# markweberdev/maskbit

Measured on AMD Instinct MI355X. Metric: images/sec (256x256, 64-step MaskBit-12bit, CFG), higher is better.
Workload: dtype f16

## Files before the change

include/maskbit_hip_diag.h:

```cpp
#ifndef MASKBIT_HIP_DIAG_H
#define MASKBIT_HIP_DIAG_H

#include "maskbit_hip.h"

#ifdef __cplusplus
extern "C" {
#endif

int mb_gemm(int epi, const void* A, const void* W, const float* bias, const float* residual, float* out_f32,
            void* out_h16, int M, int N, int K, int period, int variant, mb_stream stream);
int mb_gemm_ex(int epi, const void* A, const void* W, const float* bias, const float* residual, float* out_f32, void* out_h16,
               int M, int N, int K, const float* ln_stats, const float* ln_g, const float* ln_b, int period, int variant, mb_stream stream);
int mb_layernorm(const float* y, const float* gamma, const float* beta, float eps, float* x_f32, void* x_h16, void* x_lo, float* stats,
                 int M, int d, mb_stream stream);
int mb_gemm_act_split(int epi, const void* A_hi, const void* A_lo, const void* W, const float* bias, const float* residual,
                      float* out_f32, void* out_h16, int M, int N, int kw, int variant, mb_stream stream);
int mb_gemm_mini(int epi, const void* A, const void* W, const float* bias, const float* residual, float* out_f32, void* out_h16, void* out4,
                 void* out4_scale, int rows, int pair, int N, int K, int nlo, const void* const* lo, mb_stream stream);
int mb_gemm_mini_seq(int epi, const void* A, const void* W, const float* bias, const float* residual, float* out_f32, void* out_h16, void* out4,
                     void* out4_scale, void* out4l, void* out4l_scale, int rows, int pair, int seq_rows, int N, int K, int nlo, const void* const* lo, mb_stream stream);
int mb_w4_from_f32(const float* W, int N, int K, void* dst4, void* scale_out, mb_stream stream);
int mb_w4lo_from_f32(const float* W, int N, int K, void* dst4, void* scale_out, mb_stream stream);
int mb_gemm_head(int epi, const void* A_hi, const void* A_lo, const void* W_hi, const void* W_lo, const float* scale, const float* bias, int bias_per_pos,
                 float* out_f32, int M, int N, int kw, int period, mb_stream stream);
int mb_cast_f32_to_h16(const float* src, void* dst, int64_t n, mb_stream stream);
int mb_split_f32_planes(const float* src, void* hi, void* lo, int N, int K, float* scale_out, unsigned* tmp, mb_stream stream);
int mb_gemm_mini_split(int epi, const void* A_hi, const void* A_lo, const void* W, const float* bias, void* out_h16, void* out4, void* out4_scale,
                       int rows, int N, int kw, const void* const* lo, mb_stream stream);
int mb_gemm_mini_ln(const void* A, const void* W, const float* bias, float* y, const float* ln_stats, const float* ln_g, const float* ln_b, int rows, int pair,
                    int seq_rows, int N, int K, int nlo, const void* const* lo, mb_stream stream);
int mb_layernorm_f4(const float* y, const float* gamma, const float* beta, float eps, float* x_f32, void* x_h16, void* x4, void* x4_scale, void* xl4,
                    void* xl4_scale, int M, int d, mb_stream stream);
int mb_layernorm_f4_seq(const float* y, const float* gamma, const float* beta, float eps, float* x_f32, void* x_h16, void* x4, void* x4_scale, void* xl4,
                        void* xl4_scale, int M, int d, int seq_rows, mb_stream stream);

int mb_layernorm_pair(const float* y, const float* gamma, const float* beta, float eps, void* x_h16, float* stats, void* x4, void* x4_scale, void* xl4,
                      void* xl4_scale, int P, int d, int seq_rows, mb_stream stream);
int mb_pairify(const float* x_f32, void* x_h16, void* x4, void* x4_scale, void* xl4, void* xl4_scale, int P, int d, int seq_rows, mb_stream stream);
int mb_embed_ln(const int64_t* tokens, const int64_t* labels, const uint8_t* drop, const float* w_in, const float* b_in, const float* class_emb,
                const float* pos, const float* gamma, const float* beta, const float* tables, float* x_f32, void* x_h16, void* x_lo, void* x4,
                void* x4_scale, void* xl4, void* xl4_scale, int nb, int seq, int m, int gbits, int d, int nclass, mb_stream stream);
int mb_embed_pair(const int64_t* tokens, const int64_t* labels, const float* w_in, const float* b_in, const float* class_emb, const float* pos,
                  const float* gamma, const float* beta, const float* tables, float* x_f32, void* x_h16, void* x4, void* x4_scale, void* xl4,
                  void* xl4_scale, int nb, int seq, int m, int gbits, int d, int nclass, mb_stream stream);
int mb_attention_pair(const void* qkv, void* out_h16, int pairs, int N, int d, int heads, mb_stream stream);
int mb_attention_pair_f4(const void* qkv, void* out_h16, void* out4, void* out4_scale, void* out4l, void* out4l_scale, int pairs, int N, int d, int heads, mb_stream stream);
int mb_attention(const void* qkv, void* out_h16, void* out4, void* out4_scale, int nb, int N, int d, int heads, mb_stream stream);
int mb_attention_probs(const void* qkv, float* out_f32, int nb, int N, int d, int heads, mb_stream stream);
int mb_gen_set_alo(mb_gen* g, int gemm_mask);
int mb_set_cu_count(int n);
int mb_gen_set_walk(mb_gen* g, int mode);
int mb_diag_set_walk(int reverse);
int mb_walk_tile(int vb, int ntiles, int reverse);
int mb_walk_seq(int slot, int n, int grp, int reverse);
int mb_walk_row(int slot, int rows, int seq_rows, int pair, int reverse);
int mb_walk_group(int seq_rows, int pair);
int mb_gemm_ht_supported(int epi, int M, int N, int K);

int mb_seeded_noise(const int64_t* seeds, int step, float randomize_temperature, float conf_weight, float* exp_u, float* exp_noise, float* conf_u,
                    float* conf_noise, int B, int P, int C, mb_stream stream);

int mb_vq_argmin(const float* z, const float* codebook, int N, int C, int K, int l2, int splits, int64_t* idx, float* dist, mb_stream stream);

int mb_vq_encode_rows(const void* z_h16, int stride16, const float* z_f32, const float* codebook, int B, int HW, int C, int K, int l2, int splits,
                      int64_t* idx, float* zq_nchw, float* zraw_nchw, float* dist, mb_stream stream);
int mb_vq_gather(const int64_t* codes, const float* codebook, int64_t npix, int C, int K, int l2, int cin_pad, void* out_h16, unsigned* sat,
                 mb_stream stream);
int mb_vq_pack_latent(const float* z_nchw, int B, int K, int HW, int cin_pad, void* out_h16, unsigned* sat, mb_stream stream);
int mb_lfq_pack(const void* z_h16, int B, int HW, int K, int Kp, int64_t* idx, float* zq_nchw, float* zraw_nchw, mb_stream stream);
int mb_lfq_latent(const int64_t* tokens, int64_t npix, int K, void* out_h16, mb_stream stream);
int mb_pack_image(const float* img_nchw, int B, int C, int H, int W, void* out_h16, mb_stream stream);

int mb_conv_layer(const void* in_h16, const float* w_oihw, const float* bias, const float* gn_gamma, const float* gn_beta, const void* residual_h16,
                  void* out_h16, float* img_nchw, uint8_t* img_nhwc_u8, const float* out_gamma, const float* out_beta, float* out_scale_shift,
                  float* out_gn_part, int* part_tiles, unsigned* saturated, int B, int H, int W, int Cin, int Cout, int ks, int up, int final_layer,
                  mb_stream stream);
int mb_groupnorm_stats(const void* x_h16, const float* gamma, const float* beta, float* scale_shift, int B, int HW, int C, mb_stream stream);
int mb_avgpool2(const void* x_h16, void* y_h16, int B, int H, int W, int C, mb_stream stream);
int mb_s2d(const void* x_h16, void* y_h16, int B, int H, int W, int C, mb_stream stream);

int mb_conv_relu_layer(const void* in_h16, const float* w_oihw, const float* bias, void* out_h16, unsigned* saturated, int B, int H, int W, int Cin,
                       int Cout, int ks, mb_stream stream);
int mb_maxpool2(const void* x_h16, void* y_h16, int B, int H, int W, int C, mb_stream stream);
int mb_lpips_input(const float* real, const float* fake, const float* shift_scale, void* out_h16, int B, int H, int W, int clamp01, mb_stream stream);
int mb_lpips_distance(const void* feat_a, const void* feat_b, const float* w, int B, int HW, int C, double* per_image, mb_stream stream);
int mb_lpips_features(mb_lpips* h, const float* real, const float* fake, int B, int H, int W, int clamp01, void* tap0, void* tap1, void* tap2, void* tap3,
                      void* tap4, mb_stream stream);

int mb_convbn_layer(const void* in_h16, const float* w_oihw, const float* scale, const float* shift, void* out_h16, unsigned* saturated, int B, int H,
                    int W, int Cin, int Cout, int kh, int kw, int stride, int ph, int pw, int in_off, int in_cs, int out_off, int out_cs, int variant,
                    mb_stream stream);
int mb_pool3(const void* x_h16, void* y_h16, int B, int H, int W, int C, int mode, int in_off, int in_cs, int out_off, int out_cs, mb_stream stream);
int mb_inception_input(const uint8_t* u8, void* out_h16, int B, int H, int W, mb_stream stream);
int mb_inception_taps(mb_inception* h, const uint8_t* u8, int B, int H, int W, void* map0, void* map1, void* map2, void* map3, float* tap64,
                      float* tap192, float* tap768, float* pool, float* logits_unbiased, float* logits, mb_stream stream);

int mb_spatial_attention(const void* q, const void* k, const void* v, void* out_h16, unsigned* sat, int B, int N, int ld, int ldo, mb_stream stream);
int mb_taming_set_tap(mb_taming* h, int block, void* out_h16);

int mb_gemm_f32(int epi, const float* A, const float* W, const float* bias, const float* residual, float* out, int M, int N, int K, int period,
                int bias_per_pos, mb_stream stream);
int mb_attention_f32(const float* qkv, float* out, int nb, int N, int d, int heads, mb_stream stream);

#ifdef __cplusplus
}
#endif
#endif
```

maskbit_amd/_lib.py:

```python
from __future__ import annotations

import ctypes as C
import os
from typing import Optional

_HERE = os.path.dirname(os.path.abspath(__file__))
LIB_PATH = os.path.join(_HERE, "libmaskbit_hip.so")
ABI_VERSION = 8


class GenCfg(C.Structure):
    _fields_ = [(n, C.c_int) for n in ("bits", "splits", "hidden", "heads", "depth", "mlp", "seq", "nclass", "prenorm", "embed_tables", "precision")]


class DecCfg(C.Structure):
    _fields_ = [("token_size", C.c_int), ("hidden_channels", C.c_int), ("num_resolutions", C.c_int),
                ("num_res_blocks", C.c_int), ("num_channels", C.c_int), ("channel_mult", C.c_int * 8),
                ("latent_size", C.c_int), ("build_encoder", C.c_int), ("sample_with_conv", C.c_int),
                ("enc_res_blocks", C.c_int)]


class SamplePlan(C.Structure):
    _fields_ = [("num_steps", C.c_int), ("use_guidance", C.c_int), ("scale", C.POINTER(C.c_float)),
                ("temperature", C.POINTER(C.c_float)), ("mask_len", C.POINTER(C.c_int)), ("step_begin", C.c_int), ("step_end", C.c_int)]


class EditPlan(C.Structure):
    _fields_ = [("num_steps", C.c_int), ("use_guidance", C.c_int), ("scale", C.POINTER(C.c_float)),
                ("temperature", C.POINTER(C.c_float)), ("mask_ratio", C.POINTER(C.c_float)), ("step_begin", C.c_int), ("step_end", C.c_int)]


class RequestStep(C.Structure):
    _fields_ = [("scale", C.c_float), ("temperature", C.c_float), ("mask_ratio", C.c_float), ("randomize_temperature", C.c_float),
                ("conf_weight", C.c_float), ("step", C.c_int32)]


class RequestPlan(C.Structure):
    _fields_ = [("num_steps", C.c_int), ("use_guidance", C.c_int), ("active", C.POINTER(C.c_int)), ("table", C.c_void_p)]


SIGNATURES = {
    "mb_gen_saturation_count": (C.c_int, [C.c_void_p, C.POINTER(C.c_uint), C.c_int, C.c_void_p]),
    "mb_abi_version": (C.c_int, []),
    "mb_last_error": (C.c_char_p, []),
    "mb_gen_create": (C.c_int, [C.POINTER(GenCfg), C.c_int, C.POINTER(C.c_void_p)]),
    "mb_gen_destroy": (None, [C.c_void_p]),
    "mb_gen_load": (C.c_int, [C.c_void_p, C.c_char_p, C.c_void_p, C.POINTER(C.c_int64), C.c_int, C.c_void_p]),
    "mb_gen_set_alo": (C.c_int, [C.c_void_p, C.c_int]),
    "mb_gen_forward": (C.c_int, [C.c_void_p, C.c_void_p, C.c_void_p, C.c_void_p, C.c_void_p, C.c_int, C.c_void_p]),
    "mb_gen_forward_cfg": (C.c_int, [C.c_void_p, C.c_void_p, C.c_void_p, C.c_void_p, C.c_int, C.c_void_p]),
    "mb_gen_forward_attn": (C.c_int, [C.c_void_p, C.c_void_p, C.c_void_p, C.c_void_p, C.c_void_p, C.c_void_p, C.c_int, C.c_void_p]),
    "mb_sample_step": (C.c_int, [C.c_void_p, C.c_void_p, C.c_float, C.c_float, C.c_void_p, C.c_void_p, C.c_int,
                                 C.c_void_p, C.c_void_p, C.c_void_p, C.c_int, C.c_int, C.c_int, C.c_int, C.c_void_p]),
    "mb_dec_create": (C.c_int, [C.POINTER(DecCfg), C.c_int, C.POINTER(C.c_void_p)]),
    "mb_dec_destroy": (None, [C.c_void_p]),
    "mb_dec_load": (C.c_int, [C.c_void_p, C.c_char_p, C.c_void_p, C.POINTER(C.c_int64), C.c_int, C.c_void_p]),
    "mb_dec_decode": (C.c_int, [C.c_void_p, C.c_void_p, C.c_void_p, C.c_void_p, C.c_int, C.c_void_p]),
    "mb_dec_saturation_count": (C.c_int, [C.c_void_p, C.POINTER(C.c_uint), C.c_int, C.c_void_p]),
    "mb_enc_encode": (C.c_int, [C.c_void_p, C.c_void_p, C.c_void_p, C.c_void_p, C.c_void_p, C.c_int, C.c_void_p]),
    "mb_dec_create_vq": (C.c_int, [C.POINTER(DecCfg), C.c_int, C.c_int, C.c_int, C.POINTER(C.c_void_p)]),
    "mb_dec_decode_latent": (C.c_int, [C.c_void_p, C.c_void_p, C.c_void_p, C.c_void_p, C.c_int, C.c_void_p]),
    "mb_enc_encode_vq": (C.c_int, [C.c_void_p, C.c_void_p, C.c_void_p, C.c_void_p, C.c_void_p, C.c_void_p, C.c_int, C.c_void_p]),
    "mb_vq_argmin": (C.c_int, [C.c_void_p, C.c_void_p, C.c_int, C.c_int, C.c_int, C.c_int, C.c_int, C.c_void_p, C.c_void_p, C.c_void_p]),
    "mb_vq_encode_rows": (C.c_int, [C.c_void_p, C.c_int, C.c_void_p, C.c_void_p] + [C.c_int] * 6 + [C.c_void_p] * 5),
    "mb_vq_gather": (C.c_int, [C.c_void_p, C.c_void_p, C.c_int64, C.c_int, C.c_int, C.c_int, C.c_int, C.c_void_p, C.c_void_p, C.c_void_p]),
    "mb_vq_pack_latent": (C.c_int, [C.c_void_p, C.c_int, C.c_int, C.c_int, C.c_int, C.c_void_p, C.c_void_p, C.c_void_p]),
    "mb_lfq_pack": (C.c_int, [C.c_void_p, C.c_int, C.c_int, C.c_int, C.c_int, C.c_void_p, C.c_void_p, C.c_void_p, C.c_void_p]),
    "mb_lfq_latent": (C.c_int, [C.c_void_p, C.c_int64, C.c_int, C.c_void_p, C.c_void_p]),
    "mb_pack_image": (C.c_int, [C.c_void_p, C.c_int, C.c_int, C.c_int, C.c_int, C.c_void_p, C.c_void_p]),
    "mb_sample": (C.c_int, [C.c_void_p, C.c_void_p, C.POINTER(SamplePlan), C.c_void_p, C.c_int, C.c_void_p, C.c_void_p,
                            C.c_void_p, C.c_void_p, C.c_void_p, C.c_void_p, C.c_void_p]),
    "mb_sample_step_edit": (C.c_int, [C.c_void_p, C.c_void_p, C.c_float, C.c_float, C.c_void_p, C.c_void_p, C.c_float, C.c_void_p,
                                      C.c_void_p, C.c_void_p, C.c_void_p, C.c_int, C.c_int, C.c_int, C.c_int, C.c_void_p]),
    "mb_sample_edit": (C.c_int, [C.c_void_p, C.c_void_p, C.POINTER(EditPlan), C.c_void_p, C.c_int, C.c_void_p, C.c_void_p, C.c_void_p,
                                 C.c_void_p, C.c_void_p, C.c_void_p, C.c_void_p, C.c_void_p]),
    "mb_sample_step_seeded": (C.c_int, [C.c_void_p, C.c_void_p, C.c_float, C.c_float, C.c_void_p, C.c_int, C.c_float, C.c_float, C.c_float, C.c_void_p,
                                        C.c_void_p, C.c_void_p, C.c_void_p, C.c_int, C.c_int, C.c_int, C.c_int, C.c_void_p]),
    "mb_sample_seeded": (C.c_int, [C.c_void_p, C.c_void_p, C.POINTER(EditPlan), C.c_void_p, C.c_int, C.c_void_p, C.c_void_p, C.c_float,
                                   C.POINTER(C.c_float), C.c_void_p, C.c_void_p, C.c_void_p, C.c_void_p, C.c_void_p]),
    "mb_sample_step_requests": (C.c_int, [C.c_void_p, C.c_void_p, C.c_void_p, C.c_void_p, C.c_void_p, C.c_void_p, C.c_void_p, C.c_void_p,
                                          C.c_int, C.c_int, C.c_int, C.c_int, C.c_void_p]),
    "mb_sample_requests": (C.c_int, [C.c_void_p, C.c_void_p, C.POINTER(RequestPlan), C.c_void_p, C.c_int, C.c_void_p, C.c_void_p,
                                     C.c_void_p, C.c_void_p, C.c_void_p, C.c_void_p, C.c_void_p]),
    "mb_seeded_noise": (C.c_int, [C.c_void_p, C.c_int, C.c_float, C.c_float, C.c_void_p, C.c_void_p, C.c_void_p, C.c_void_p, C.c_int, C.c_int, C.c_int,
                                  C.c_void_p]),
    "mb_edit_init": (C.c_int, [C.c_void_p, C.c_void_p, C.c_void_p, C.c_void_p, C.c_int, C.c_int, C.c_int, C.c_int, C.c_void_p]),
    "mb_edit_token_mask": (C.c_int, [C.c_void_p, C.c_void_p, C.c_int, C.c_int, C.c_int, C.c_int, C.c_void_p]),
    "mb_edit_composite": (C.c_int, [C.c_void_p, C.c_void_p, C.c_void_p, C.c_void_p, C.c_void_p, C.c_int, C.c_int, C.c_int, C.c_int, C.c_void_p]),
    "mb_gemm_ex": (C.c_int, [C.c_int, C.c_void_p, C.c_void_p, C.c_void_p, C.c_void_p, C.c_void_p, C.c_void_p, C.c_int, C.c_int, C.c_int,
                             C.c_void_p, C.c_void_p, C.c_void_p, C.c_int, C.c_int, C.c_void_p]),
    "mb_layernorm": (C.c_int, [C.c_void_p, C.c_void_p, C.c_void_p, C.c_float, C.c_void_p, C.c_void_p, C.c_void_p, C.c_void_p, C.c_int, C.c_int, C.c_void_p]),
    "mb_w4_from_f32": (C.c_int, [C.c_void_p, C.c_int, C.c_int, C.c_void_p, C.c_void_p, C.c_void_p]),
    "mb_w4lo_from_f32": (C.c_int, [C.c_void_p, C.c_int, C.c_int, C.c_void_p, C.c_void_p, C.c_void_p]),
    "mb_gemm_head": (C.c_int, [C.c_int, C.c_void_p, C.c_void_p, C.c_void_p, C.c_void_p, C.c_void_p, C.c_void_p, C.c_int, C.c_void_p, C.c_int, C.c_int,
                               C.c_int, C.c_int, C.c_void_p]),
    "mb_cast_f32_to_h16": (C.c_int, [C.c_void_p, C.c_void_p, C.c_int64, C.c_void_p]),
    "mb_split_f32_planes": (C.c_int, [C.c_void_p, C.c_void_p, C.c_void_p, C.c_int, C.c_int, C.c_void_p, C.c_void_p, C.c_void_p]),
    "mb_layernorm_f4": (C.c_int, [C.c_void_p, C.c_void_p, C.c_void_p, C.c_float, C.c_void_p, C.c_void_p, C.c_void_p, C.c_void_p, C.c_void_p, C.c_void_p,
                                  C.c_int, C.c_int, C.c_void_p]),
    "mb_layernorm_f4_seq": (C.c_int, [C.c_void_p, C.c_void_p, C.c_void_p, C.c_float] + [C.c_void_p] * 6 + [C.c_int] * 3 + [C.c_void_p]),
    "mb_layernorm_pair": (C.c_int, [C.c_void_p, C.c_void_p, C.c_void_p, C.c_float] + [C.c_void_p] * 6 + [C.c_int] * 3 + [C.c_void_p]),
    "mb_pairify": (C.c_int, [C.c_void_p] * 6 + [C.c_int] * 3 + [C.c_void_p]),
    "mb_embed_ln": (C.c_int, [C.c_void_p] * 17 + [C.c_int] * 6 + [C.c_void_p]),
    "mb_embed_pair": (C.c_int, [C.c_void_p] * 15 + [C.c_int] * 6 + [C.c_void_p]),
    "mb_attention": (C.c_int, [C.c_void_p, C.c_void_p, C.c_void_p, C.c_void_p, C.c_int, C.c_int, C.c_int, C.c_int, C.c_void_p]),
    "mb_attention_probs": (C.c_int, [C.c_void_p, C.c_void_p, C.c_int, C.c_int, C.c_int, C.c_int, C.c_void_p]),
    "mb_attention_pair": (C.c_int, [C.c_void_p, C.c_void_p, C.c_int, C.c_int, C.c_int, C.c_int, C.c_void_p]),
    "mb_attention_pair_f4": (C.c_int, [C.c_void_p, C.c_void_p, C.c_void_p, C.c_void_p, C.c_void_p, C.c_void_p, C.c_int, C.c_int, C.c_int, C.c_int, C.c_void_p]),
    "mb_gemm_mini": (C.c_int, [C.c_int, C.c_void_p, C.c_void_p, C.c_void_p, C.c_void_p, C.c_void_p, C.c_void_p, C.c_void_p, C.c_void_p, C.c_int, C.c_int,
                               C.c_int, C.c_int, C.c_int, C.POINTER(C.c_void_p), C.c_void_p]),
    "mb_gemm_mini_seq": (C.c_int, [C.c_int, C.c_void_p, C.c_void_p, C.c_void_p, C.c_void_p, C.c_void_p, C.c_void_p, C.c_void_p, C.c_void_p, C.c_void_p, C.c_void_p, C.c_int, C.c_int,
                                   C.c_int, C.c_int, C.c_int, C.c_int, C.POINTER(C.c_void_p), C.c_void_p]),
    "mb_gemm_mini_split": (C.c_int, [C.c_int, C.c_void_p, C.c_void_p, C.c_void_p, C.c_void_p, C.c_void_p, C.c_void_p, C.c_void_p, C.c_int, C.c_int, C.c_int,
                                     C.POINTER(C.c_void_p), C.c_void_p]),
    "mb_gemm_mini_ln": (C.c_int, [C.c_void_p] * 7 + [C.c_int] * 6 + [C.POINTER(C.c_void_p), C.c_void_p]),
    "mb_gemm_act_split": (C.c_int, [C.c_int, C.c_void_p, C.c_void_p, C.c_void_p, C.c_void_p, C.c_void_p, C.c_void_p, C.c_void_p, C.c_int, C.c_int, C.c_int,
                                    C.c_int, C.c_void_p]),
    "mb_gemm": (C.c_int, [C.c_int, C.c_void_p, C.c_void_p, C.c_void_p, C.c_void_p, C.c_void_p, C.c_void_p, C.c_int, C.c_int, C.c_int,
                          C.c_int, C.c_int, C.c_void_p]),
    "mb_conv_layer": (C.c_int, [C.c_void_p] * 13 + [C.POINTER(C.c_int), C.POINTER(C.c_uint)] + [C.c_int] * 8 + [C.c_void_p]),
    "mb_groupnorm_stats": (C.c_int, [C.c_void_p, C.c_void_p, C.c_void_p, C.c_void_p, C.c_int, C.c_int, C.c_int, C.c_void_p]),
    "mb_avgpool2": (C.c_int, [C.c_void_p, C.c_void_p, C.c_int, C.c_int, C.c_int, C.c_int, C.c_void_p]),
    "mb_s2d": (C.c_int, [C.c_void_p, C.c_void_p, C.c_int, C.c_int, C.c_int, C.c_int, C.c_void_p]),
    "mb_eval_workspace_bytes": (C.c_size_t, [C.c_int, C.c_int, C.c_int, C.c_int]),
    "mb_eval_images": (C.c_int, [C.c_void_p, C.c_void_p, C.c_int, C.c_int, C.c_int, C.c_int, C.c_uint, C.c_int, C.c_void_p, C.c_void_p, C.c_void_p, C.c_void_p]),
    "mb_eval_codebook": (C.c_int, [C.c_void_p, C.c_int64, C.c_int, C.c_void_p, C.c_void_p, C.c_void_p]),
    "mb_mlm_workspace_bytes": (C.c_size_t, [C.c_int, C.c_int, C.c_int, C.c_int]),
    "mb_mlm_state_bytes": (C.c_size_t, []),
    "mb_mlm_mask": (C.c_int, [C.c_void_p, C.c_void_p, C.c_void_p, C.c_int64, C.c_void_p, C.c_void_p, C.c_int, C.c_int, C.c_int, C.c_void_p]),
    "mb_mlm_loss": (C.c_int, [C.c_void_p, C.c_void_p, C.c_void_p, C.c_float, C.c_int, C.c_int, C.c_int, C.c_int, C.c_void_p, C.c_void_p, C.c_void_p,
                              C.c_void_p, C.c_void_p]),
    "mb_lpips_create": (C.c_int, [C.c_int, C.c_int, C.c_int, C.POINTER(C.c_void_p)]),
    "mb_lpips_destroy": (None, [C.c_void_p]),
    "mb_lpips_load": (C.c_int, [C.c_void_p, C.c_char_p, C.c_void_p, C.POINTER(C.c_int64), C.c_int, C.c_void_p]),
    "mb_lpips_forward": (C.c_int, [C.c_void_p, C.c_void_p, C.c_void_p, C.c_int, C.c_int, C.c_int, C.c_int, C.c_void_p, C.c_void_p, C.c_void_p]),
    "mb_lpips_saturation_count": (C.c_int, [C.c_void_p, C.POINTER(C.c_uint), C.c_int, C.c_void_p]),
    "mb_conv_relu_layer": (C.c_int, [C.c_void_p] * 4 + [C.POINTER(C.c_uint)] + [C.c_int] * 6 + [C.c_void_p]),
    "mb_maxpool2": (C.c_int, [C.c_void_p, C.c_void_p, C.c_int, C.c_int, C.c_int, C.c_int, C.c_void_p]),
    "mb_lpips_input": (C.c_int, [C.c_void_p, C.c_void_p, C.c_void_p, C.c_void_p, C.c_int, C.c_int, C.c_int, C.c_int, C.c_void_p]),
    "mb_lpips_distance": (C.c_int, [C.c_void_p, C.c_void_p, C.c_void_p, C.c_int, C.c_int, C.c_int, C.c_void_p, C.c_void_p]),
    "mb_lpips_features": (C.c_int, [C.c_void_p, C.c_void_p, C.c_void_p, C.c_int, C.c_int, C.c_int, C.c_int] + [C.c_void_p] * 6),
    "mb_fid_accumulate": (C.c_int, [C.c_void_p, C.c_int, C.c_int, C.c_int, C.c_int64, C.c_void_p, C.c_void_p, C.c_void_p]),
    "mb_is_workspace_bytes": (C.c_size_t, [C.c_int, C.c_int]),
    "mb_is_accumulate": (C.c_int, [C.c_void_p, C.c_int, C.c_int, C.c_int, C.c_int64, C.c_void_p, C.c_void_p, C.c_void_p, C.c_void_p]),
    "mb_manifold_workspace_bytes": (C.c_size_t, [C.c_int, C.c_int]),
    "mb_knn_radii": (C.c_int, [C.c_void_p, C.c_int, C.c_int, C.c_int, C.c_int64, C.c_int, C.c_void_p, C.c_void_p, C.c_void_p]),
    "mb_manifold_cover": (C.c_int, [C.c_void_p, C.c_int, C.c_int, C.c_int64, C.c_void_p, C.c_int, C.c_int, C.c_int64, C.c_int, C.c_void_p, C.c_void_p,
                                    C.c_void_p, C.c_void_p]),
    "mb_inception_create": (C.c_int, [C.c_int, C.POINTER(C.c_void_p)]),
    "mb_inception_destroy": (None, [C.c_void_p]),
    "mb_inception_load": (C.c_int, [C.c_void_p, C.c_char_p, C.c_void_p, C.POINTER(C.c_int64), C.c_int, C.c_void_p]),
    "mb_inception_forward": (C.c_int, [C.c_void_p, C.c_void_p, C.c_int, C.c_int, C.c_int, C.c_void_p, C.c_void_p, C.c_void_p, C.c_void_p]),
    "mb_inception_forward_spatial": (C.c_int, [C.c_void_p, C.c_void_p, C.c_int, C.c_int, C.c_int, C.c_void_p, C.c_void_p, C.c_void_p, C.c_void_p, C.c_void_p]),
    "mb_inception_saturation_count": (C.c_int, [C.c_void_p, C.POINTER(C.c_uint), C.c_int, C.c_void_p]),
    "mb_convbn_layer": (C.c_int, [C.c_void_p] * 5 + [C.POINTER(C.c_uint)] + [C.c_int] * 15 + [C.c_void_p]),
    "mb_pool3": (C.c_int, [C.c_void_p, C.c_void_p] + [C.c_int] * 9 + [C.c_void_p]),
    "mb_inception_input": (C.c_int, [C.c_void_p, C.c_void_p, C.c_int, C.c_int, C.c_int, C.c_void_p]),
    "mb_inception_taps": (C.c_int, [C.c_void_p, C.c_void_p, C.c_int, C.c_int, C.c_int] + [C.c_void_p] * 11),
    "mb_taming_create": (C.c_int, [C.c_int, C.c_int, C.POINTER(C.c_void_p)]),
    "mb_taming_destroy": (None, [C.c_void_p]),
    "mb_taming_load": (C.c_int, [C.c_void_p, C.c_char_p, C.c_void_p, C.POINTER(C.c_int64), C.c_int, C.c_void_p]),
    "mb_taming_encode": (C.c_int, [C.c_void_p, C.c_void_p, C.c_void_p, C.c_void_p, C.c_void_p, C.c_void_p, C.c_int, C.c_void_p]),
    "mb_taming_decode": (C.c_int, [C.c_void_p, C.c_void_p, C.c_void_p, C.c_void_p, C.c_int, C.c_void_p]),
    "mb_taming_decode_latent": (C.c_int, [C.c_void_p, C.c_void_p, C.c_void_p, C.c_void_p, C.c_int, C.c_void_p]),
    "mb_taming_saturation_count": (C.c_int, [C.c_void_p, C.POINTER(C.c_uint), C.c_int, C.c_void_p]),
    "mb_taming_set_tap": (C.c_int, [C.c_void_p, C.c_int, C.c_void_p]),
    "mb_spatial_attention": (C.c_int, [C.c_void_p] * 5 + [C.c_int] * 4 + [C.c_void_p]),
    "mb_gemm_f32": (C.c_int, [C.c_int] + [C.c_void_p] * 5 + [C.c_int] * 5 + [C.c_void_p]),
    "mb_attention_f32": (C.c_int, [C.c_void_p, C.c_void_p] + [C.c_int] * 4 + [C.c_void_p]),
    "mb_set_cu_count":(C.c_int, [C.c_int]),
    "mb_gen_set_walk": (C.c_int, [C.c_void_p, C.c_int]),
    "mb_diag_set_walk": (C.c_int, [C.c_int]),
    "mb_walk_tile": (C.c_int, [C.c_int] * 3),
    "mb_walk_seq": (C.c_int, [C.c_int] * 4),
    "mb_walk_row": (C.c_int, [C.c_int] * 5),
    "mb_walk_group": (C.c_int, [C.c_int] * 2),
    "mb_gemm_ht_supported": (C.c_int, [C.c_int, C.c_int, C.c_int, C.c_int]),
    "mb_prof_enable": (C.c_int, [C.c_int]),
    "mb_prof_read": (C.c_int, [C.c_char_p, C.c_int]),
}

_lib: Optional[C.CDLL] = None


def load() -> C.CDLL:
    global _lib
    if _lib is not None:
        return _lib
    import torch
    if not os.path.exists(LIB_PATH):
        raise RuntimeError(
            f"{LIB_PATH} is missing: the MaskBit HIP kernels are not built. Run `python -c 'import __graft_entry__ as g; "
            f"g.build()'` (needs hipcc, gfx950). There is no CPU fallback in maskbit_amd.")
    lib = C.CDLL(LIB_PATH)
    for name, (res, args) in SIGNATURES.items():
        fn = getattr(lib, name)
        fn.restype = res
        fn.argtypes = args
    v = lib.mb_abi_version()
    if v != ABI_VERSION:
        raise RuntimeError(f"libmaskbit_hip.so ABI {v} != binding ABI {ABI_VERSION}; rebuild")
    _lib = lib
    return lib


def check(rc: int, what: str = "") -> None:
    if rc != 0:
        msg = load().mb_last_error()
        raise RuntimeError(f"{what or 'libmaskbit_hip'} failed (code {rc}): {msg.decode() if msg else '?'}")


def prof_enable(on, every: int = 1) -> None:
    load().mb_prof_enable(max(1, int(every)) if on else 0)


def prof_read() -> dict:
    buf = C.create_string_buffer(1 << 16)
    n = load().mb_prof_read(buf, len(buf))
    if n < 0:
        check(n, "mb_prof_read")
    out = {}
    for line in buf.value.decode().splitlines():
        name, calls, ms = line.split()
        out[name] = (int(calls), float(ms))
    return out
```

maskbit_amd/build.py:

```python
from __future__ import annotations

import os
import shutil
import subprocess
import sys

HERE = os.path.dirname(os.path.abspath(__file__))
CSRC = os.path.join(HERE, "csrc")
LIB = os.path.join(HERE, "libmaskbit_hip.so")
SOURCES = ["engine.hip", "diag.hip", "gemm.hip", "gemm_ht.hip", "gemm_f32.hip", "norm_embed.hip", "attention.hip", "sampling.hip", "edit.hip", "conv.hip", "decoder.hip", "vq.hip", "evaluator.hip", "mlm.hip", "lpips.hip", "fid.hip", "manifold.hip", "inception.hip", "spatial_attention.hip", "taming.hip"]


def hipcc() -> str:
    for cand in (os.environ.get("HIPCC"), shutil.which("hipcc"), "/opt/rocm/bin/hipcc"):
        if cand and os.path.exists(cand):
            return cand
    raise RuntimeError("hipcc not found (needed to build the gfx950 kernels)")


def needs_build(lib: str = LIB) -> bool:
    if not os.path.exists(lib):
        return True
    t = os.path.getmtime(lib)
    inc = os.path.join(HERE, "..", "include")
    deps = [os.path.join(CSRC, f) for f in os.listdir(CSRC)] + [os.path.join(inc, "maskbit_hip.h"), os.path.join(inc, "maskbit_hip_diag.h")]
    return any(os.path.getmtime(p) > t for p in deps)


def build(force: bool = False, verbose: bool = False) -> str:
    if not force and not needs_build():
        return LIB
    objs = []
    flags = ["--offload-arch=gfx950", "-O3", "-std=c++17", "-fPIC", "-Wno-unused-result"]
    procs = []
    bdir = os.path.join(HERE, "build")
    os.makedirs(bdir, exist_ok=True)
    for src in SOURCES:
        obj = os.path.join(bdir, src.replace(".hip", ".o"))
        objs.append(obj)
        cmd = [hipcc(), *flags, "-c", os.path.join(CSRC, src), "-o", obj]
        if verbose:
            print(" ".join(cmd))
        procs.append((src, subprocess.Popen(cmd, stdout=subprocess.PIPE, stderr=subprocess.STDOUT, text=True)))
    for src, p in procs:
        out, _ = p.communicate()
        if p.returncode != 0:
            raise RuntimeError(f"hipcc failed on {src}:\n{out}")
        if verbose and out.strip():
            print(out)
    cmd = [hipcc(), "--offload-arch=gfx950", "-shared", "-fPIC", *objs, "-o", LIB]
    r = subprocess.run(cmd, stdout=subprocess.PIPE, stderr=subprocess.STDOUT, text=True)
    if r.returncode != 0:
        raise RuntimeError(f"link failed:\n{r.stdout}")
    return LIB


if __name__ == "__main__":
    print(build(force="--force" in sys.argv, verbose=True))
```

maskbit_amd/csrc/engine.hip:

```cpp
#include <hip/hip_runtime.h>

#include <algorithm>
#include <cstdio>
#include <cstring>
#include <string>
#include <vector>

#include "../../include/maskbit_hip_diag.h"
#include "mb_abi.h"
#include "mb_kernels.h"

using mb::fail;
using mb::g_prof;
using mb::launched;
using mb::ProfScope;

struct F4Buf { uint8_t *v = nullptr, *s = nullptr; };

struct mb_gen {
  mb_gen_cfg c{};
  int max_seqs = 0, chunk_seqs = 0, N = 0, C = 0, gbits = 0, device = 0;
  struct Layer {
    h16 *wqkv = nullptr, *wo = nullptr, *w1 = nullptr, *w2 = nullptr;
    float *bqkv = nullptr, *bo = nullptr, *b1 = nullptr, *b2 = nullptr;
    float *ln1g = nullptr, *ln1b = nullptr, *ln2g = nullptr, *ln2b = nullptr;
  };
  std::vector<Layer> layers;
  float *w_in = nullptr, *b_in = nullptr, *class_emb = nullptr, *pos = nullptr, *ln0g = nullptr, *ln0b = nullptr;
  h16 *wl = nullptr, *wp = nullptr;
  float *bl = nullptr, *lnhg = nullptr, *lnhb = nullptr, *bp = nullptr;
  float *lnag = nullptr, *lnab = nullptr;
  float *tables = nullptr, *bias_pos = nullptr;
  unsigned* split_tmp = nullptr;
  float *y_f32 = nullptr, *ln_stats = nullptr;
  h16 *x_h16 = nullptr, *x_lo = nullptr, *qkv = nullptr, *att = nullptr, *h = nullptr;
  bool pair_ok = false, mini_ok = false;
  F4Buf x4, xl4;
  std::vector<uint8_t*> w4, w4s;
  float* logits_tmp = nullptr;
  h16 *wl_lo = nullptr, *wp_lo = nullptr;
  float* head_scale = nullptr;
  unsigned* sat = nullptr;
  std::vector<uint8_t*> w4lo, w4los;
  F4Buf att4, h4;
  F4Buf attl4, hl4;
  struct Run {
    struct Id {
      int B = 0, steps = 0, guided = 0, kind = 0;
      bool operator==(const Id& o) const { return B == o.B && steps == o.steps && guided == o.guided && kind == o.kind; }
    } id;
    int next = -1;
    const int64_t* cfg_labels = nullptr;
    int cfg_B = 0;
  } run;
  int* num_regen = nullptr;
  int alo_mask = 0, alo_mask_built = 0;
  int walk = 1;
  bool f32 = false;
  struct Layer32 { float *wqkv = nullptr, *wo = nullptr, *w1 = nullptr, *w2 = nullptr; };
  std::vector<Layer32> layers32;
  float *wl32 = nullptr, *wp32 = nullptr;
  float *x_f32 = nullptr, *qkv32 = nullptr, *att32 = nullptr, *h32 = nullptr;
  int64_t *tok_a = nullptr, *tok_b = nullptr, *tok_cfg = nullptr, *lab_cfg = nullptr, *pred = nullptr, *codes = nullptr;
  uint8_t* drop_cfg = nullptr;
  float* logits = nullptr;
  mb::DevArena mem;
  int loaded = 0;
};

namespace {

void alloc_f4(mb::DevArena& m, F4Buf* b, size_t rows, size_t width, size_t ntok) {
  m.zeroed(&b->v, rows * 2 * width);
  m.zeroed(&b->s, (width / 64) * ntok + 256);
}

int head_gemms(mb_gen* g, float* logits, int M, hipStream_t s) {
  using namespace mb;
  const mb_gen_cfg& c = g->c;
  const int d = c.hidden;
  int rc = 0;
  { ProfScope p("gemm_head", s, true);
    GemmArgs ga{g->x_h16, g->wl, g->bl, nullptr, g->y_f32, nullptr, M, d, 3 * d, 0, g->head_scale};
    ga.A2 = g->x_lo; ga.kw = d; ga.W2 = g->wl_lo;
    rc |= gemm_tn(s, EPI_GELU_F32, ga); }
  { ProfScope p("layernorm", s, true);
    layernorm_rows(s, g->y_f32, g->lnhg, g->lnhb, 1e-12f, nullptr, g->x_h16, nullptr, M, d, g->x_lo); }
  { ProfScope p("gemm_head", s, true);
    GemmArgs ga{g->x_h16, g->wp, c.embed_tables ? g->bias_pos : g->bp, nullptr, logits, nullptr, M, c.splits * g->C, (g->wp_lo ? 3 : 2) * d, g->N,
                g->wp_lo ? g->head_scale + 1 : nullptr};
    ga.A2 = g->x_lo; ga.kw = d; ga.W2 = g->wp_lo;
    ga.bias_per_pos = c.embed_tables;
    rc |= gemm_tn(s, EPI_LOGITS_F32, ga); }
  return rc;
}

int gen_forward_impl(mb_gen* g, const int64_t* tokens, const int64_t* labels, const uint8_t* drop, float* logits,
                     int nb, hipStream_t s, float* attn = nullptr) {
  using namespace mb;
  const mb_gen_cfg& c = g->c;
  const int d = c.hidden, f = c.mlp, N = g->N, M = nb * N;
  auto attn_maps = [&](int l) {
    return attn ? attention_probs(s, g->qkv, attn + (size_t)l * nb * N * N, nb, N, d, c.heads) : 0;
  };
  int attn_rc = 0, gemm_rc = 0;
  int wdir = 0;
  auto walk_next = [&] { wdir ^= g->walk; return wdir; };
  const bool xlo = c.precision >= 1;
  const bool wm = g->mini_ok && c.precision >= 2;
  const bool xlo_all = xlo && !wm;
  auto xlo_layer = [&](int l) { return xlo && (xlo_all || 2 * l + 1 >= c.depth); };
  h16* const xlo_ffn = xlo ? g->x_lo : nullptr;
  h16* const xlo_qkv = xlo_all ? g->x_lo : nullptr;
  Fp4Rows f4x;
  if (wm) { f4x.x4 = g->x4.v; f4x.x4s = g->x4.s; f4x.nseq = nb; f4x.seq_rows = N; }
  auto lo_set = [&](GemmArgs& ga, const uint8_t* a4, const uint8_t* a4s, int widx) {
    if (!wm) return;
    ga.nlo = 1; ga.lo[0] = {a4, a4s, g->w4lo[widx], g->w4los[widx]};
  };
  auto xgemm = [&](GemmEpi epi, const h16* W, const float* bias, h16* out, int Nout, int widx) {
    GemmArgs ga{g->x_h16, W, bias, nullptr, nullptr, out, M, Nout, d, 0};
    if (wm) ga.seq_rows = N;
    lo_set(ga, g->x4.v, g->x4.s, widx);
    if (wm && epi == EPI_GELU_H16) { ga.out4 = g->h4.v; ga.out4_scale = g->h4.s; }
    if (((widx & 3) == 2 || xlo_all) && xlo_layer(widx >> 2)) { ga.K = 2 * d; ga.A2 = g->x_lo; ga.kw = d; }
    ga.sat = g->sat;
    ga.reverse = walk_next();
    gemm_rc |= gemm_tn(s, epi, ga, wm ? 257 : 0);
  };
  auto rgemm = [&](const h16* A, const h16* W, const float* bias, int K, int widx, const uint8_t* a4, const uint8_t* a4s, const float* ln_g, const float* ln_b) {
    GemmArgs ga{A, W, bias, g->y_f32, g->y_f32, nullptr, M, d, K, 0};
    if (ln_g) { ga.ln_stats = g->ln_stats; ga.ln_g = ln_g; ga.ln_b = ln_b; }
    if (wm) ga.seq_rows = N;
    lo_set(ga, a4, a4s, widx);
    ga.reverse = walk_next();
    gemm_rc |= gemm_tn(s, EPI_RES_F32, ga, wm ? 257 : 0);
  };
  {
    ProfScope p("embed_ln", s, true);
    EmbedArgs e{tokens, labels, drop, g->w_in, g->b_in, g->class_emb, g->pos, g->ln0g, g->ln0b,
                g->y_f32, g->x_h16, nb, c.seq, c.splits, g->gbits, d, c.nclass, g->tables};
    e.x_lo = c.depth ? (c.prenorm ? nullptr : xlo_qkv) : g->x_lo;
    e.f4 = f4x;
    embed_ln(s, e);
  }
  for (int l = 0; l < c.depth; ++l) {
    const mb_gen::Layer& L = g->layers[l];
    if (c.prenorm) { ProfScope p("layernorm", s, true); layernorm_rows(s, g->y_f32, L.ln1g, L.ln1b, 1e-12f, nullptr, g->x_h16, nullptr, M, d, xlo_qkv, f4x, walk_next(), N); }
    { ProfScope p("gemm_qkv", s, true); xgemm(EPI_H16, L.wqkv, L.bqkv, g->qkv, 3 * d, 4 * l); }
    { ProfScope p("attention", s, true); attention(s, g->qkv, g->att, nb, N, d, c.heads, wm ? g->att4.v : nullptr, wm ? g->att4.s : nullptr, walk_next()); }
    attn_rc |= attn_maps(l);
    { ProfScope p("gemm_attn_out", s, true);
      const bool re = !c.prenorm && l > 0;
      rgemm(g->att, L.wo, L.bo, d, 4 * l + 1, g->att4.v, g->att4.s, re ? g->layers[l - 1].ln2g : nullptr, re ? g->layers[l - 1].ln2b : nullptr); }
    { ProfScope p("layernorm", s, true);
      layernorm_rows(s, g->y_f32, c.prenorm ? L.ln2g : L.ln1g, c.prenorm ? L.ln2b : L.ln1b, 1e-12f, nullptr, g->x_h16, c.prenorm ? nullptr : g->ln_stats, M, d, xlo_layer(l) ? xlo_ffn : nullptr, f4x, walk_next(), N); }
    { ProfScope p("gemm_ffn_up", s, true); xgemm(EPI_GELU_H16, L.w1, L.b1, g->h, f, 4 * l + 2); }
    { ProfScope p("gemm_ffn_down", s, true);
      rgemm(g->h, L.w2, L.b2, f, 4 * l + 3, g->h4.v, g->h4.s, c.prenorm ? nullptr : L.ln1g, c.prenorm ? nullptr : L.ln1b); }
    if (!c.prenorm) { ProfScope p("layernorm", s, true);
      const bool last = l + 1 == c.depth;
      layernorm_rows(s, g->y_f32, L.ln2g, L.ln2b, 1e-12f, nullptr, g->x_h16, g->ln_stats, M, d, last ? g->x_lo : xlo_qkv, last ? Fp4Rows{} : f4x, walk_next(), N); }
  }
  if (c.prenorm) { ProfScope p("layernorm", s, true); layernorm_rows(s, g->y_f32, g->lnag, g->lnab, 1e-12f, nullptr, g->x_h16, nullptr, M, d, g->x_lo, Fp4Rows{}, walk_next(), N); }
  gemm_rc |= head_gemms(g, logits, M, s);
  if (int rc = launched()) return rc;
  if (attn_rc) return fail(-3, "attention maps: head dim %d / %d tokens not supported", d / c.heads, N);
  if (gemm_rc) return fail(-3, "a trunk GEMM of this forward (%d sequences x %d tokens, hidden %d, mlp %d; precision %d%s) is outside the half-tile "
                               "kernel's shapes: its correction mini-tiles cannot run", nb, N, d, f, c.precision, wm ? ", weight-correction mini-tiles" : "");
  return 0;
}

int gen_forward_pair_impl(mb_gen* g, const int64_t* tokens, const int64_t* labels, const uint8_t* drop, float* logits, int B, bool wmode, hipStream_t s) {
  using namespace mb;
  const mb_gen_cfg& c = g->c;
  const int d = c.hidden, f = c.mlp, N = g->N, nb = 2 * B, M = nb * N, P = B * N;
  int rc = 0;
  int wdir = 0;
  auto walk_next = [&] { wdir ^= g->walk; return wdir; };
  auto alo_on = [&](int gemm) { return wmode && c.precision >= 3 && ((g->alo_mask >> gemm) & 1); };
  auto f4_for = [&](bool feeds_ffn = false) {
    Fp4Rows f;
    if (wmode) {
      f.x4 = g->x4.v; f.x4s = g->x4.s; f.nseq = B; f.seq_rows = N;
      if (alo_on(feeds_ffn ? 2 : 0)) { f.xl4 = g->xl4.v; f.xl4s = g->xl4.s; }
    }
    return f;
  };
  auto pgemm = [&](GemmEpi epi, const h16* A, const h16* W, const float* bias, h16* out16, float* res, int Nout, int K, int widx, int lo,
                   const uint8_t* a4 = nullptr, const uint8_t* a4s = nullptr, const uint8_t* al4 = nullptr, const uint8_t* al4s = nullptr) {
    GemmArgs ga{A, W, bias, res, res, out16, M, Nout, K, 0};
    ga.pair_rows = P;
    ga.seq_rows = N;
    if (epi != EPI_RES_F32) ga.sat = g->sat;
    if (lo) {
      ga.nlo = lo; ga.lo[0] = {a4, a4s, g->w4lo[widx], g->w4los[widx]};
      if (lo == 2) ga.lo[1] = {al4, al4s, g->w4[widx], g->w4s[widx]};
    }
    ga.reverse = walk_next();
    return ga;
  };
  {
    ProfScope p("embed_ln", s, true);
    EmbedArgs e{tokens, labels, nullptr, g->w_in, g->b_in, g->class_emb, g->pos, g->ln0g, g->ln0b,
                g->y_f32, g->x_h16, B, c.seq, c.splits, g->gbits, d, c.nclass, g->tables};
    e.f4 = f4_for();
    if (embed_pair(s, e)) {
      e.drop = drop; e.nb = nb; e.f4 = Fp4Rows{};
      embed_ln(s, e);
      rc |= pairify_rows(s, g->y_f32, g->x_h16, P, d, f4_for(), walk_next(), N);
    }
  }
  if (c.prenorm && c.depth > 0) {
    ProfScope p("layernorm", s, true);
    rc |= layernorm_pair(s, g->y_f32, g->layers[0].ln1g, g->layers[0].ln1b, 1e-12f, g->x_h16, nullptr, P, d, f4_for(), walk_next(), N);
  }
  for (int l = 0; l < c.depth; ++l) {
    const mb_gen::Layer& L = g->layers[l];
    const int xlo_mode = wmode ? (alo_on(2) ? 2 : 1) : 0;
    { ProfScope p("gemm_qkv", s, true);
      GemmArgs ga = pgemm(EPI_H16, g->x_h16, L.wqkv, L.bqkv, g->qkv, nullptr, 3 * d, d, 4 * l, wmode ? (alo_on(0) ? 2 : 1) : 0, g->x4.v, g->x4.s, g->xl4.v, g->xl4.s);
      rc |= gemm_tn(s, EPI_H16, ga, 257); }
    const bool lo_o = alo_on(1), lo_h = alo_on(3);
    { ProfScope p("attention", s, true); rc |= attention_pair(s, g->qkv, g->att, B, N, d, c.heads, wmode ? g->att4.v : nullptr, wmode ? g->att4.s : nullptr,
                                                              lo_o ? g->attl4.v : nullptr, lo_o ? g->attl4.s : nullptr, walk_next()); }
    { ProfScope p("gemm_attn_out", s, true);
      GemmArgs ga = pgemm(EPI_RES_F32, g->att, L.wo, L.bo, nullptr, g->y_f32, d, d, 4 * l + 1, wmode ? (alo_on(1) ? 2 : 1) : 0, g->att4.v, g->att4.s, g->attl4.v, g->attl4.s);
      if (l > 0 && !c.prenorm) { ga.ln_stats = g->ln_stats; ga.ln_g = g->layers[l - 1].ln2g; ga.ln_b = g->layers[l - 1].ln2b; }
      rc |= gemm_tn(s, EPI_RES_F32, ga, 257); }
    { ProfScope p("layernorm", s, true);
      rc |= layernorm_pair(s, g->y_f32, c.prenorm ? L.ln2g : L.ln1g, c.prenorm ? L.ln2b : L.ln1b, 1e-12f, g->x_h16, c.prenorm ? nullptr : g->ln_stats, P, d, f4_for(true), walk_next(), N); }
    { ProfScope p("gemm_ffn_up", s, true);
      GemmArgs ga = pgemm(EPI_GELU_H16, g->x_h16, L.w1, L.b1, g->h, nullptr, f, d, 4 * l + 2, xlo_mode, g->x4.v, g->x4.s, g->xl4.v, g->xl4.s);
      if (wmode) { ga.out4 = g->h4.v; ga.out4_scale = g->h4.s; }
      if (lo_h) { ga.out4l = g->hl4.v; ga.out4l_scale = g->hl4.s; }
      rc |= gemm_tn(s, EPI_GELU_H16, ga, 257); }
    { ProfScope p("gemm_ffn_down", s, true);
      GemmArgs ga = pgemm(EPI_RES_F32, g->h, L.w2, L.b2, nullptr, g->y_f32, d, f, 4 * l + 3, wmode ? (alo_on(3) ? 2 : 1) : 0, g->h4.v, g->h4.s, g->hl4.v, g->hl4.s);
      if (!c.prenorm) { ga.ln_stats = g->ln_stats; ga.ln_g = L.ln1g; ga.ln_b = L.ln1b; }
      rc |= gemm_tn(s, EPI_RES_F32, ga, 257); }
    { ProfScope p("layernorm", s, true);
      if (c.prenorm) {
        if (l + 1 == c.depth) layernorm_rows(s, g->y_f32, g->lnag, g->lnab, 1e-12f, nullptr, g->x_h16, nullptr, M, d, g->x_lo, Fp4Rows{}, walk_next(), N);
        else rc |= layernorm_pair(s, g->y_f32, g->layers[l + 1].ln1g, g->layers[l + 1].ln1b, 1e-12f, g->x_h16, nullptr, P, d, f4_for(), walk_next(), N);
      }
      else if (l + 1 == c.depth) layernorm_rows(s, g->y_f32, L.ln2g, L.ln2b, 1e-12f, nullptr, g->x_h16, g->ln_stats, M, d, g->x_lo, Fp4Rows{}, walk_next(), N);
      else rc |= layernorm_pair(s, g->y_f32, L.ln2g, L.ln2b, 1e-12f, g->x_h16, g->ln_stats, P, d, f4_for(), walk_next(), N); }
  }
  rc |= head_gemms(g, logits, M, s);
  if (int lrc = launched()) return lrc;
  if (rc) return fail(-3, "differential CFG forward: a kernel refused the shape (%d pairs x %d tokens, hidden %d, mlp %d)", B, N, d, f);
  return 0;
}

int gen_forward_f32_impl(mb_gen* g, const int64_t* tokens, const int64_t* labels, const uint8_t* drop, float* logits, int nb, hipStream_t s) {
  using namespace mb;
  const mb_gen_cfg& c = g->c;
  const int d = c.hidden, f = c.mlp, N = g->N, M = nb * N;
  int rc = 0;
  auto gemm = [&](int epi, const float* A, const float* W, const float* bias, const float* res, float* out, int Nout, int K) {
    GemmF32Args ga{epi, A, W, bias, res, out, M, Nout, K};
    rc |= gemm_f32(s, ga);
  };
  auto ln = [&](const float* gamma, const float* beta) {
    ProfScope p("layernorm", s, true);
    layernorm_rows(s, g->y_f32, gamma, beta, 1e-12f, g->x_f32, nullptr, nullptr, M, d);
  };
  float* const stream = c.prenorm ? g->y_f32 : g->x_f32;
  {
    ProfScope p("embed_ln", s, true);
    EmbedArgs e{tokens, labels, drop, g->w_in, g->b_in, g->class_emb, g->pos, g->ln0g, g->ln0b,
                stream, nullptr, nb, c.seq, c.splits, g->gbits, d, c.nclass, g->tables};
    embed_ln(s, e);
  }
  for (int l = 0; l < c.depth; ++l) {
    const mb_gen::Layer& L = g->layers[l];
    const mb_gen::Layer32& W = g->layers32[l];
    if (c.prenorm) ln(L.ln1g, L.ln1b);
    { ProfScope p("gemm_qkv", s, true); gemm(F32_EPI_PLAIN, g->x_f32, W.wqkv, L.bqkv, nullptr, g->qkv32, 3 * d, d); }
    { ProfScope p("attention", s, true); rc |= attention_f32(s, g->qkv32, g->att32, nb, N, d, c.heads); }
    { ProfScope p("gemm_attn_out", s, true); gemm(F32_EPI_RES, g->att32, W.wo, L.bo, stream, g->y_f32, d, d); }
    ln(c.prenorm ? L.ln2g : L.ln1g, c.prenorm ? L.ln2b : L.ln1b);
    { ProfScope p("gemm_ffn_up", s, true); gemm(F32_EPI_GELU, g->x_f32, W.w1, L.b1, nullptr, g->h32, f, d); }
    { ProfScope p("gemm_ffn_down", s, true); gemm(F32_EPI_RES, g->h32, W.w2, L.b2, stream, g->y_f32, d, f); }
    if (!c.prenorm) ln(L.ln2g, L.ln2b);
  }
  if (c.prenorm) ln(g->lnag, g->lnab);
  { ProfScope p("gemm_head", s, true); gemm(F32_EPI_GELU, g->x_f32, g->wl32, g->bl, nullptr, g->y_f32, d, d); }
  ln(g->lnhg, g->lnhb);
  { ProfScope p("gemm_head", s, true);
    GemmF32Args ga{F32_EPI_LOGITS, g->x_f32, g->wp32, c.embed_tables ? g->bias_pos : g->bp, nullptr, logits, M, c.splits * g->C, d, N, c.embed_tables};
    rc |= gemm_f32(s, ga); }
  if (int lrc = launched()) return lrc;
  if (rc) return fail(-3, "fp32 reference forward: a kernel refused the shape (%d sequences x %d tokens, hidden %d, heads %d, mlp %d)", nb, N, d, c.heads, f);
  return 0;
}

int gen_forward_pass(mb_gen* g, const int64_t* tokens, const int64_t* labels, const uint8_t* drop, float* logits, int nb, hipStream_t s, float* attn = nullptr) {
  if (g->f32) return gen_forward_f32_impl(g, tokens, labels, drop, logits, nb, s);
  return gen_forward_impl(g, tokens, labels, drop, logits, nb, s, attn);
}

int gen_forward(mb_gen* g, const int64_t* tokens, const int64_t* labels, const uint8_t* drop, float* logits, int nb, hipStream_t s,
                float* attn = nullptr) {
  const int chunk = g->chunk_seqs;
  g_prof.begin_forward(true);
  if (nb <= chunk) return gen_forward_pass(g, tokens, labels, drop, logits, nb, s, attn);
  if (attn) return fail(-3, "attention maps are limited to %d sequences per call", chunk);
  const size_t P = (size_t)g->c.seq * g->c.splits;
  for (int b0 = 0; b0 < nb; b0 += chunk) {
    const int nc = nb - b0 < chunk ? nb - b0 : chunk;
    int rc = gen_forward_pass(g, tokens + (size_t)b0 * P, labels + b0, drop ? drop + b0 : nullptr, logits + (size_t)b0 * P * g->C, nc, s);
    if (rc) return rc;
  }
  return 0;
}

int gen_forward_cfg(mb_gen* g, const int64_t* tokens, const int64_t* labels, float* logits, int B, hipStream_t s) {
  const size_t P = (size_t)g->c.seq * g->c.splits;
  const bool pair = !g->f32 && g->pair_ok && g->c.precision >= 1;
  const bool wmode = pair && g->c.precision >= 2;
  const int chunk = g->chunk_seqs / 2;
  if (chunk < 1) return fail(-1, "engine holds %d sequences: too few for a guided forward", g->chunk_seqs);
  for (int b0 = 0; b0 < B; b0 += chunk) {
    const int nc = B - b0 < chunk ? B - b0 : chunk;
    HIP_TRY(hipMemcpyAsync(g->tok_cfg, tokens + (size_t)b0 * P, nc * P * sizeof(int64_t), hipMemcpyDeviceToDevice, s));
    if (!(pair && !g->c.embed_tables && g->c.bits <= 24))
      HIP_TRY(hipMemcpyAsync(g->tok_cfg + nc * P, tokens + (size_t)b0 * P, nc * P * sizeof(int64_t), hipMemcpyDeviceToDevice, s));
    if (!(nc == B && g->run.cfg_labels == labels && g->run.cfg_B == B)) {
      HIP_TRY(hipMemcpyAsync(g->lab_cfg, labels + b0, nc * sizeof(int64_t), hipMemcpyDeviceToDevice, s));
      HIP_TRY(hipMemcpyAsync(g->lab_cfg + nc, labels + b0, nc * sizeof(int64_t), hipMemcpyDeviceToDevice, s));
      HIP_TRY(hipMemsetAsync(g->drop_cfg, 0, nc, s));
      HIP_TRY(hipMemsetAsync(g->drop_cfg + nc, 1, nc, s));
    }
    float* out = (nc == B) ? logits : g->logits_tmp;
    if (b0 == 0) g_prof.begin_forward(false);
    int rc = pair ? gen_forward_pair_impl(g, g->tok_cfg, g->lab_cfg, g->drop_cfg, out, nc, wmode, s)
                  : gen_forward_pass(g, g->tok_cfg, g->lab_cfg, g->drop_cfg, out, 2 * nc, s);
    if (rc) return rc;
    if (nc != B) {
      HIP_TRY(hipMemcpyAsync(logits + (size_t)b0 * P * g->C, out, nc * P * g->C * sizeof(float), hipMemcpyDeviceToDevice, s));
      HIP_TRY(hipMemcpyAsync(logits + (size_t)(B + b0) * P * g->C, out + (size_t)nc * P * g->C, nc * P * g->C * sizeof(float), hipMemcpyDeviceToDevice, s));
    }
  }
  return 0;
}

}

extern "C" {

int mb_abi_version(void) { return MB_ABI_VERSION; }
const char* mb_last_error(void) { return mb::g_err.c_str(); }

int mb_prof_enable(int on) {
  if (!on) g_prof.drain();
  g_prof.on = on != 0;
  if (on) { g_prof.acc.clear(); g_prof.stride = on; g_prof.tick[0] = g_prof.tick[1] = 0; }
  return 0;
}
int mb_prof_read(char* buf, int buflen) {
  g_prof.drain();
  std::string out;
  char line[256];
  for (auto& kv : g_prof.acc) {
    snprintf(line, sizeof line, "%s %ld %.6f\n", g_prof.names[kv.first].c_str(), kv.second.first, kv.second.second);
    out += line;
  }
  if ((int)out.size() + 1 > buflen) return fail(-3, "mb_prof_read: buffer too small (%zu needed)", out.size() + 1);
  memcpy(buf, out.c_str(), out.size() + 1);
  return (int)out.size();
}

int mb_gen_create(const mb_gen_cfg* cfg, int max_seqs, mb_gen** out) {
  if (!cfg || !out || max_seqs <= 0) return fail(-1, "mb_gen_create: bad arguments");
  const mb_gen_cfg& c = *cfg;
  if (c.splits <= 0 || c.bits % c.splits) return fail(-1, "bits (%d) must be divisible by splits (%d)", c.bits, c.splits);
  if (c.bits > 24) return fail(-1, "bits > 24 is not supported");
  if (c.hidden % 64 || c.mlp % 64) return fail(-1, "hidden (%d) and mlp (%d) must be multiples of 64", c.hidden, c.mlp);
  if (c.hidden > 2048) return fail(-1, "hidden > 2048 is not supported");
  const int dh = c.heads > 0 ? c.hidden / c.heads : 0;
  if (c.heads <= 0 || c.hidden % c.heads || (dh != 32 && dh != 64)) return fail(-1, "hidden/heads must be 32 or 64 (got %d)", dh);
  if (c.seq < 1 || c.seq > 4096) return fail(-1, "seq = %d outside [1, 4096]", c.seq);
  if ((size_t)c.seq * c.splits > 8192) return fail(-1, "seq * splits = %zu exceeds the step kernel's 8192 positions", (size_t)c.seq * c.splits);
  const int C = 1 << (c.bits / c.splits);
  if (C > 4096 || (c.splits * C) % 4) return fail(-1, "unsupported group codebook size %d (the fused step kernel holds up to 4096 codes per group)", C);
  if ((c.prenorm != 0 && c.prenorm != 1) || (c.embed_tables != 0 && c.embed_tables != 1)) return fail(-1, "prenorm / embed_tables must be 0 or 1");
  if (c.embed_tables && c.splits > 8) return fail(-1, "embed_tables supports up to 8 token groups");
  if (c.precision < 0 || c.precision > MB_PREC_F32) return fail(-1, "precision must be 0 .. 5 (MB_PREC_FP16 / _DIFF / _WCORR / _ALO / _ALO_ALL / _F32)");
  const bool f32 = c.precision == MB_PREC_F32;
  mb_gen* g = new mb_gen();
  g->f32 = f32;
  g->c = c; g->max_seqs = max_seqs; g->N = c.seq + 1; g->gbits = c.bits / c.splits; g->C = C;
  (void)hipGetDevice(&g->device);
  const size_t widest = (size_t)(c.mlp > 3 * c.hidden ? c.mlp : 3 * c.hidden);
  const size_t max_rows = ((1ull << 32) - 1) / (4 * widest);
  g->chunk_seqs = (int)std::min<size_t>((size_t)max_seqs, std::max<size_t>(1, max_rows / g->N));
  const size_t d = c.hidden, f = c.mlp, M = (size_t)g->chunk_seqs * g->N;
  mb::DevArena& m = g->mem;
  g->layers.resize(c.depth);
  if (f32) g->layers32.resize(c.depth);
  else m.get(&g->split_tmp, 1);
  m.zeroed(&g->sat, 1);
  for (int l = 0; l < c.depth; ++l) {
    mb_gen::Layer& L = g->layers[l];
    if (f32) { mb_gen::Layer32& W = g->layers32[l]; m.get(&W.wqkv, 3 * d * d); m.get(&W.wo, d * d); m.get(&W.w1, f * d); m.get(&W.w2, d * f); }
    else { m.get(&L.wqkv, 3 * d * d); m.get(&L.wo, d * d); m.get(&L.w1, f * d); m.get(&L.w2, d * f); }
    m.get(&L.bqkv, 3 * d); m.get(&L.bo, d); m.get(&L.b1, f); m.get(&L.b2, d);
    m.get(&L.ln1g, d); m.get(&L.ln1b, d); m.get(&L.ln2g, d); m.get(&L.ln2b, d);
  }
  m.get(&g->w_in, d * c.bits); m.get(&g->b_in, d);
  if (c.prenorm) { m.get(&g->lnag, d); m.get(&g->lnab, d); }
  if (c.embed_tables) { m.get(&g->tables, (size_t)c.splits * (C + 1) * d); m.get(&g->bias_pos, (size_t)c.seq * c.splits * C); }
  m.get(&g->class_emb, (size_t)(c.nclass + 1) * d); m.get(&g->pos, (size_t)g->N * d);
  m.get(&g->ln0g, d); m.get(&g->ln0b, d);
  m.get(&g->bl, d); m.get(&g->lnhg, d); m.get(&g->lnhb, d); m.get(&g->bp, (size_t)c.splits * C);
  m.get(&g->y_f32, M * d);
  if (f32) {
    m.get(&g->wl32, d * d); m.get(&g->wp32, (size_t)c.splits * C * d);
    m.get(&g->x_f32, M * d); m.get(&g->qkv32, M * 3 * d); m.get(&g->att32, M * d); m.get(&g->h32, M * f);
  } else {
    m.get(&g->wl, d * d); m.get(&g->wl_lo, d * d);
    m.get(&g->wp, (size_t)c.splits * C * d); m.get(&g->head_scale, 2);
    if (!c.embed_tables) m.get(&g->wp_lo, (size_t)c.splits * C * d);
    m.get(&g->ln_stats, M * 2); m.get(&g->x_h16, M * d);
    m.get(&g->x_lo, M * d);
    m.get(&g->qkv, M * 3 * d); m.get(&g->att, M * d); m.get(&g->h, M * f);
  }
  g->mini_ok = !f32 && c.precision >= 2 && (c.seq == 256 || c.seq == 1024) && (c.hidden == 768 || c.hidden == 1024) && c.mlp % 256 == 0 && c.hidden / c.heads == 64;
  if (c.precision == 3) g->alo_mask = g->alo_mask_built = 6;
  if (c.precision == 4) g->alo_mask = g->alo_mask_built = 14;
  g->pair_ok = !f32 && c.precision >= 1 && (c.seq == 256 || c.seq == 1024) && (c.hidden == 768 || c.hidden == 1024) && c.mlp % 256 == 0 && g->chunk_seqs >= 2 &&
               (c.precision == 1 || g->mini_ok);
  if (g->mini_ok) {
    const size_t ntok = (size_t)g->chunk_seqs * c.seq;
    alloc_f4(m, &g->x4, M, d, ntok);
    alloc_f4(m, &g->att4, M, d, ntok);
    alloc_f4(m, &g->h4, M, f, ntok);
    if (g->alo_mask_built & 5) alloc_f4(m, &g->xl4, M, d, ntok);
    if (g->alo_mask_built & 2) alloc_f4(m, &g->attl4, M, d, ntok);
    if (g->alo_mask_built & 8) alloc_f4(m, &g->hl4, M, f, ntok);
    g->w4lo.assign((size_t)4 * c.depth, nullptr); g->w4los.assign((size_t)4 * c.depth, nullptr);
    g->w4.assign((size_t)4 * c.depth, nullptr); g->w4s.assign((size_t)4 * c.depth, nullptr);
    const size_t wn[4] = {3 * d * d, d * d, f * d, d * f};
    for (int i = 0; i < 4 * c.depth; ++i) {
      const size_t n = wn[i & 3];
      m.get(&g->w4lo[i], n / 2); m.get(&g->w4los[i], n / 128);
      if ((g->alo_mask_built >> (i & 3)) & 1) { m.get(&g->w4[i], n / 2); m.get(&g->w4s[i], n / 128); }
    }
  }
  const size_t P = (size_t)c.seq * c.splits, B = max_seqs;
  m.get(&g->tok_a, B * P); m.get(&g->tok_b, B * P); m.get(&g->tok_cfg, B * P);
  m.get(&g->pred, B * P); m.get(&g->codes, B * c.seq);
  m.get(&g->lab_cfg, B); m.get(&g->drop_cfg, B); m.get(&g->logits, B * P * C);
  m.get(&g->num_regen, B);
  if (g->chunk_seqs < max_seqs) m.get(&g->logits_tmp, (size_t)g->chunk_seqs * P * C);
  if (int rc = m.failed("mb_gen_create")) { delete g; return rc; }
  *out = g;
  return 0;
}

void mb_gen_destroy(mb_gen* g) { delete g; }

int mb_gen_load(mb_gen* g, const char* name, const float* data, const int64_t* shape, int ndim, mb_stream stream) {
  if (!g || !name || !data) return fail(-1, "mb_gen_load: bad arguments");
  hipStream_t s = (hipStream_t)stream;
  const mb_gen_cfg& c = g->c;
  const size_t d = c.hidden, f = c.mlp;
  size_t numel = 1;
  for (int i = 0; i < ndim; ++i) numel *= (size_t)shape[i];
  float* dst_f = nullptr; h16* dst_h = nullptr; size_t want = 0;
  int wrows = 0, wcols = 0, sidx = -1;
  int l = -1, sub = -1; char rest[96] = {0};
  std::string n(name);
  if (c.embed_tables && (n.rfind("prediction_layer.", 0) == 0 || n.rfind("input_proj.", 0) == 0))
    return fail(-2, "mb_gen_load: unknown checkpoint entry '%s' (embed_tables engine: tok_emb_list.* / bias.* instead)", name);
  if (sscanf(name, "transformer.layers.%d.%d.%95s", &l, &sub, rest) == 3) {
    if (l < 0 || l >= c.depth) return fail(-2, "layer index out of range in '%s'", name);
    mb_gen::Layer& L = g->layers[l];
    std::string r(rest);
    if (sub == 0) {
      if (r == "mha.in_proj_weight") { dst_h = L.wqkv; want = 3 * d * d; wrows = 3 * d; wcols = d; sidx = 4 * l; }
      else if (r == "mha.in_proj_bias") { dst_f = L.bqkv; want = 3 * d; }
      else if (r == "mha.out_proj.weight") { dst_h = L.wo; want = d * d; wrows = d; wcols = d; sidx = 4 * l + 1; }
      else if (r == "mha.out_proj.bias") { dst_f = L.bo; want = d; }
      else if (r == "norm.weight") { dst_f = L.ln1g; want = d; }
      else if (r == "norm.bias") { dst_f = L.ln1b; want = d; }
    } else if (sub == 1) {
      if (r == "net.0.weight") { dst_h = L.w1; want = f * d; wrows = f; wcols = d; sidx = 4 * l + 2; }
      else if (r == "net.0.bias") { dst_f = L.b1; want = f; }
      else if (r == "net.2.weight") { dst_h = L.w2; want = d * f; wrows = d; wcols = f; sidx = 4 * l + 3; }
      else if (r == "net.2.bias") { dst_f = L.b2; want = d; }
      else if (r == "norm.weight") { dst_f = L.ln2g; want = d; }
      else if (r == "norm.bias") { dst_f = L.ln2b; want = d; }
    }
  } else if (n == "pos_emb") { dst_f = g->pos; want = (size_t)g->N * d; }
  else if (n == "class_emb.weight") { dst_f = g->class_emb; want = (size_t)(c.nclass + 1) * d; }
  else if (n == "input_proj.weight") { dst_f = g->w_in; want = d * c.bits; }
  else if (n == "input_proj.bias") { dst_f = g->b_in; want = d; }
  else if (n == "first_layer.0.weight") { dst_f = g->ln0g; want = d; }
  else if (n == "first_layer.0.bias") { dst_f = g->ln0b; want = d; }
  else if (n == "last_layer.0.weight") { dst_h = g->wl; want = d * d; wrows = d; wcols = d; sidx = 4 * c.depth; }
  else if (n == "last_layer.0.bias") { dst_f = g->bl; want = d; }
  else if (n == "last_layer.2.weight") { dst_f = g->lnhg; want = d; }
  else if (n == "last_layer.2.bias") { dst_f = g->lnhb; want = d; }
  else if (n == "prediction_layer.weight") { dst_h = g->wp; want = (size_t)c.splits * g->C * d; wrows = c.splits * g->C; wcols = d; sidx = 4 * c.depth + 1; }
  else if (n == "prediction_layer.bias") { dst_f = g->bp; want = (size_t)c.splits * g->C; }
  else if (n == "bits_to_indices") return 0;
  else if (c.prenorm && n == "norm_after_transformer.weight") { dst_f = g->lnag; want = d; }
  else if (c.prenorm && n == "norm_after_transformer.bias") { dst_f = g->lnab; want = d; }
  else if (c.embed_tables) {
    int q = -1;
    if (sscanf(name, "tok_emb_list.%d.weight", &q) == 1 && n == "tok_emb_list." + std::to_string(q) + ".weight") {
      if (q < 0 || q >= c.splits) return fail(-2, "group index out of range in '%s'", name);
      const size_t rows = (size_t)g->C + 1;
      if (numel != rows * d) return fail(-4, "mb_gen_load: '%s' has %zu elements, expected %zu", name, numel, rows * d);
      HIP_TRY(hipMemcpyAsync(g->tables + (size_t)q * rows * d, data, numel * sizeof(float), hipMemcpyDeviceToDevice, s));
      if (g->f32) HIP_TRY(hipMemcpyAsync(g->wp32 + (size_t)q * g->C * d, data, (size_t)g->C * d * sizeof(float), hipMemcpyDeviceToDevice, s));
      else mb::cast_f32_to_h16(s, data, g->wp + (size_t)q * g->C * d, (size_t)g->C * d);
      g->loaded++;
      return 0;
    }
    if (sscanf(name, "bias.%d", &q) == 1 && n == "bias." + std::to_string(q)) {
      if (q < 0 || q >= c.splits) return fail(-2, "group index out of range in '%s'", name);
      if (numel != (size_t)c.seq * g->C) return fail(-4, "mb_gen_load: '%s' has %zu elements, expected %zu", name, numel, (size_t)c.seq * g->C);
      HIP_TRY(hipMemcpy2DAsync(g->bias_pos + (size_t)q * g->C, (size_t)c.splits * g->C * sizeof(float), data, (size_t)g->C * sizeof(float),
                               (size_t)g->C * sizeof(float), (size_t)c.seq, hipMemcpyDeviceToDevice, s));
      g->loaded++;
      return 0;
    }
  }
  if (g->f32 && sidx >= 0) {
    if (sidx < 4 * c.depth) { mb_gen::Layer32& W = g->layers32[sidx >> 2]; float* const w4[4] = {W.wqkv, W.wo, W.w1, W.w2}; dst_f = w4[sidx & 3]; }
    else dst_f = sidx == 4 * c.depth ? g->wl32 : g->wp32;
    dst_h = nullptr;
  }
  if (!dst_f && !dst_h) return fail(-2, "mb_gen_load: unknown checkpoint entry '%s'", name);
  if (numel != want) return fail(-4, "mb_gen_load: '%s' has %zu elements, expected %zu", name, numel, want);
  if (dst_f == g->w_in) mb::transpose_f32(s, data, g->w_in, (int)d, c.bits);
  else if (dst_h && dst_h == g->wl) mb::split_f32_to_h16_planes(s, data, g->wl, g->wl_lo, wrows, wcols, g->head_scale, g->split_tmp);
  else if (dst_h && dst_h == g->wp) mb::split_f32_to_h16_planes(s, data, g->wp, g->wp_lo, wrows, wcols, g->head_scale + 1, g->split_tmp);
  else if (dst_h) {
    mb::cast_f32_to_h16(s, data, dst_h, numel);
    if (g->mini_ok && sidx >= 0 && sidx < 4 * c.depth) {
      mb::w4lo_from_f32(s, data, g->w4lo[sidx], wrows, wcols, g->w4los[sidx]);
      if (g->w4[sidx]) mb::w4_from_f32(s, data, g->w4[sidx], wrows, wcols, g->w4s[sidx]);
    }
  }
  else HIP_TRY(hipMemcpyAsync(dst_f, data, numel * sizeof(float), hipMemcpyDeviceToDevice, s));
  g->loaded++;
  return 0;
}

int mb_gen_set_alo(mb_gen* g, int gemm_mask) {
  if (!g || gemm_mask < 0 || gemm_mask > 15) return fail(-1, "mb_gen_set_alo: mask outside [0, 15]");
  if (gemm_mask & ~g->alo_mask_built)
    return fail(-1, "mb_gen_set_alo: the handle was created (precision %d) with the activation-lo operands of GEMM mask %d only", g->c.precision, g->alo_mask_built);
  g->alo_mask = gemm_mask;
  return 0;
}

int mb_gen_set_walk(mb_gen* g, int mode) {
  if (!g || (mode != 0 && mode != 1)) return fail(-1, "mb_gen_set_walk: mode 0 (every launch front to back) or 1 (alternating)");
  g->walk = mode;
  return 0;
}

int mb_gen_saturation_count(mb_gen* g, unsigned* count, int reset, mb_stream stream) {
  if (!g || !count) return fail(-1, "mb_gen_saturation_count: null argument");
  HIP_TRY(hipMemcpyAsync(count, g->sat, sizeof(unsigned), hipMemcpyDeviceToHost, (hipStream_t)stream));
  if (reset) HIP_TRY(hipMemsetAsync(g->sat, 0, sizeof(unsigned), (hipStream_t)stream));
  HIP_TRY(hipStreamSynchronize((hipStream_t)stream));
  return 0;
}

int mb_gen_forward(mb_gen* g, const int64_t* tokens, const int64_t* labels, const uint8_t* drop, float* logits,
                   int nb, mb_stream stream) {
  if (!g || !tokens || !labels || !logits) return fail(-1, "mb_gen_forward: null argument");
  if (nb <= 0 || nb > g->max_seqs) return fail(-1, "mb_gen_forward: nb=%d outside [1, %d]", nb, g->max_seqs);
  return gen_forward(g, tokens, labels, drop, logits, nb, (hipStream_t)stream);
}

int mb_gen_forward_cfg(mb_gen* g, const int64_t* tokens, const int64_t* labels, float* logits, int B, mb_stream stream) {
  if (!g || !tokens || !labels || !logits) return fail(-1, "mb_gen_forward_cfg: null argument");
  if (B <= 0 || 2 * B > g->max_seqs) return fail(-1, "mb_gen_forward_cfg: B=%d needs %d sequences, engine holds %d", B, 2 * B, g->max_seqs);
  return gen_forward_cfg(g, tokens, labels, logits, B, (hipStream_t)stream);
}

int mb_gen_forward_attn(mb_gen* g, const int64_t* tokens, const int64_t* labels, const uint8_t* drop, float* logits, float* attn,
                        int nb, mb_stream stream) {
  if (!g || !tokens || !labels || !logits || !attn) return fail(-1, "mb_gen_forward_attn: null argument");
  if (nb <= 0 || nb > g->max_seqs) return fail(-1, "mb_gen_forward_attn: nb=%d outside [1, %d]", nb, g->max_seqs);
  if (g->f32) return fail(-3, "mb_gen_forward_attn: attention maps are not available in the fp32 reference mode (precision %d)", (int)MB_PREC_F32);
  return gen_forward(g, tokens, labels, drop, logits, nb, (hipStream_t)stream, attn);
}

static int sample_step_checked(const char* who, const mb::StepArgs& a, const int64_t* tokens_in, const int32_t* num_regen, float mask_ratio, hipStream_t s) {
  if (!a.logits_c || (!a.seeds && (!a.exp_noise || !a.conf_noise)) || !tokens_in || !a.tokens) return fail(-1, "%s: null argument", who);
  if (tokens_in == a.tokens) return fail(-1, "%s: tokens_in and tokens_out must not alias", who);
  if (a.B <= 0 || a.P <= 0 || a.C <= 0) return fail(-1, "%s: bad sizes", who);
  ProfScope p(a.req ? "sample_step_requests" : a.seeds ? "sample_step_seeded" : num_regen ? "sample_step_edit" : "sample_step", s);
  if (mb::sample_step(s, a, tokens_in, num_regen, mask_ratio)) return fail(-1, "%s: C=%d or n*m=%d too large", who, a.C, a.P);
  return launched();
}

static int step_slots(int n, int m) { return n > 0 && m > 0 ? n * m : 0; }

int mb_sample_step(const float* logits_c, const float* logits_u, float scale, float temperature,
                   const float* exp_noise, const float* conf_noise, int k_mask_len, const int64_t* tokens_in,
                   int64_t* tokens_out, int64_t* pred_out, int B, int n, int m, int C, mb_stream stream) {
  mb::StepArgs a{};
  a.logits_c = logits_c; a.logits_u = logits_u; a.scale = scale; a.temperature = temperature;
  a.exp_noise = exp_noise; a.conf_noise = conf_noise; a.k_mask_len = k_mask_len;
  a.tokens = tokens_out; a.pred = pred_out; a.B = B; a.P = step_slots(n, m); a.C = C;
  return sample_step_checked("mb_sample_step", a, tokens_in, nullptr, 0.f, (hipStream_t)stream);
}

int mb_sample_step_edit(const float* logits_c, const float* logits_u, float scale, float temperature, const float* exp_noise, const float* conf_noise,
                        float mask_ratio, const int32_t* num_regen, const int64_t* tokens_in, int64_t* tokens_out, int64_t* pred_out, int B, int n, int m,
                        int C, mb_stream stream) {
  if (!num_regen) return fail(-1, "mb_sample_step_edit: null argument");
  mb::StepArgs a{};
  a.logits_c = logits_c; a.logits_u = logits_u; a.scale = scale; a.temperature = temperature;
  a.exp_noise = exp_noise; a.conf_noise = conf_noise;
  a.tokens = tokens_out; a.pred = pred_out; a.B = B; a.P = step_slots(n, m); a.C = C;
  return sample_step_checked("mb_sample_step_edit", a, tokens_in, num_regen, mask_ratio, (hipStream_t)stream);
}

int mb_sample_step_seeded(const float* logits_c, const float* logits_u, float scale, float temperature, const int64_t* seeds, int step,
                          float randomize_temperature, float conf_weight, float mask_ratio, const int32_t* num_regen, const int64_t* tokens_in,
                          int64_t* tokens_out, int64_t* pred_out, int B, int n, int m, int C, mb_stream stream) {
  if (!seeds || !num_regen) return fail(-1, "mb_sample_step_seeded: null argument");
  if (step < 0) return fail(-1, "mb_sample_step_seeded: step = %d is negative", step);
  if (pred_out && (pred_out == tokens_out || pred_out == tokens_in)) return fail(-1, "mb_sample_step_seeded: pred_out must not alias tokens_in or tokens_out");
  mb::StepArgs a{};
  a.logits_c = logits_c; a.logits_u = logits_u; a.scale = scale; a.temperature = temperature;
  a.seeds = seeds; a.step = step; a.rand_temp = randomize_temperature; a.conf_w = conf_weight;
  a.tokens = tokens_out; a.pred = pred_out; a.B = B; a.P = step_slots(n, m); a.C = C;
  return sample_step_checked("mb_sample_step_seeded", a, tokens_in, num_regen, mask_ratio, (hipStream_t)stream);
}

static_assert(sizeof(mb::RequestStep) == sizeof(mb_request_step) && sizeof(mb_request_step) == 24, "mb_request_step is the kernels' RequestStep");

int mb_sample_step_requests(const float* logits_c, const float* logits_u, const mb_request_step* table_row, const int64_t* seeds, const int32_t* num_regen,
                            const int64_t* tokens_in, int64_t* tokens_out, int64_t* pred_out, int B, int n, int m, int C, mb_stream stream) {
  if (!table_row || !seeds || !num_regen) return fail(-1, "mb_sample_step_requests: null argument");
  if (pred_out && (pred_out == tokens_out || pred_out == tokens_in)) return fail(-1, "mb_sample_step_requests: pred_out must not alias tokens_in or tokens_out");
  mb::StepArgs a{};
  a.logits_c = logits_c; a.logits_u = logits_u;
  a.seeds = seeds; a.req = (const mb::RequestStep*)table_row;
  a.tokens = tokens_out; a.pred = pred_out; a.B = B; a.P = step_slots(n, m); a.C = C;
  return sample_step_checked("mb_sample_step_requests", a, tokens_in, num_regen, 0.f, (hipStream_t)stream);
}

}

namespace {

struct RunNoise {
  const float* exp_noise = nullptr; const float* conf_noise = nullptr;
  const int64_t* seeds = nullptr; float rand_temp = 0.f; const float* conf_weight = nullptr;
};
struct RunSpec {
  const char* who = nullptr;
  int num_steps = 0, use_guidance = 0, step_begin = 0, step_end = 0;
  const float* scale = nullptr; const float* temperature = nullptr;
  const int* mask_len = nullptr; const float* mask_ratio = nullptr;
  const int64_t* init_tokens = nullptr;
  RunNoise noise;
};
struct RunOut { int64_t* step_tokens; int64_t* codes; float* img_nchw; uint8_t* img_nhwc_u8; };

const char* const kRunKind[3] = {"plain", "edit", "seeded"};
const char* const kStepEntry[3] = {"mb_sample_step", "mb_sample_step_edit", "mb_sample_step_seeded"};

template <class Plan>
RunSpec run_spec(const char* who, const Plan& p) {
  RunSpec r;
  r.who = who; r.num_steps = p.num_steps; r.use_guidance = p.use_guidance; r.step_begin = p.step_begin; r.step_end = p.step_end;
  r.scale = p.scale; r.temperature = p.temperature;
  return r;
}

int sample_run(mb_gen* g, mb_dec* d, const RunSpec& r, const int64_t* labels, int B, const RunOut& out, hipStream_t s) {
  const char* who = r.who;
  const RunNoise& nz = r.noise;
  const bool edit = r.mask_ratio != nullptr, seeded = nz.seeds != nullptr;
  const int num_steps = r.num_steps;
  if (!r.scale || !r.temperature || !(edit ? (const void*)r.mask_ratio : (const void*)r.mask_len) || num_steps <= 0) return fail(-1, "%s: incomplete plan", who);
  const mb_gen::Run::Id id{B, num_steps, r.use_guidance != 0, seeded ? 2 : edit ? 1 : 0};
  const int nbf = id.guided ? 2 * B : B;
  if (B <= 0 || nbf > g->max_seqs) return fail(-1, "%s: B=%d needs %d sequences, engine holds %d", who, B, nbf, g->max_seqs);
  if (!d && (out.img_nchw || out.img_nhwc_u8)) return fail(-1, "%s: image requested without a decoder", who);
  const mb_gen_cfg& c = g->c;
  const int n = c.seq, m = c.splits, C = g->C;
  const size_t P = (size_t)n * m;
  const int s0 = r.step_end > 0 ? r.step_begin : 0, s1 = r.step_end > 0 ? r.step_end : num_steps;
  if (s0 < 0 || s1 > num_steps || s0 >= s1) return fail(-1, "%s: step chunk [%d, %d) outside [0, %d)", who, s0, s1, num_steps);
  mb_gen::Run& run = g->run;
  if (s0 == 0) {
    if (r.init_tokens) mb::edit_load_tokens(s, r.init_tokens, g->tok_a, g->num_regen, B, (int)P, C);
    else {
      mb::fill_i64(s, g->tok_a, (int64_t)C, (size_t)B * P);
      if (seeded) mb::edit_load_tokens(s, g->tok_a, nullptr, g->num_regen, B, (int)P, C);
    }
    run.id = id;
  }
  else if (!(run.id == id && run.next == s0))
    return fail(-1, "%s: step chunk [%d, %d) of a %d-step %s run with B = %d does not continue the run in progress (next step %d of %d, B = %d, %s %s run)",
                who, s0, s1, num_steps, kRunKind[id.kind], B, run.next, run.id.steps, run.id.B, run.id.kind == 1 ? "an" : "a", kRunKind[run.id.kind]);
  run.next = -1;
  int64_t* cur = (s0 & 1) ? g->tok_b : g->tok_a;
  int64_t* nxt = (s0 & 1) ? g->tok_a : g->tok_b;
  int64_t* last_pred = g->pred;
  struct CfgReady { mb_gen::Run& run; ~CfgReady() { run.cfg_labels = nullptr; } } cfg_ready{run};
  run.cfg_labels = nullptr;
  mb::StepArgs a{};
  a.logits_c = g->logits; a.B = B; a.P = (int)P; a.C = C;
  a.seeds = nz.seeds; a.rand_temp = nz.rand_temp;
  for (int i = s0; i < s1; ++i) {
    int rc;
    if (id.guided && (r.scale[i] != 0.0f || (!g->f32 && g->pair_ok && c.precision >= 4))) {
      rc = gen_forward_cfg(g, cur, labels, g->logits, B, s);
      a.logits_u = g->logits + (size_t)B * P * C;
      if (B <= g->chunk_seqs / 2) { run.cfg_labels = labels; run.cfg_B = B; }
    } else {
      rc = gen_forward(g, cur, labels, nullptr, g->logits, B, s);
      a.logits_u = nullptr;
    }
    if (rc) return rc;
    const size_t k = (size_t)(i - s0);
    a.scale = r.scale[i]; a.temperature = r.temperature[i];
    a.tokens = nxt; a.pred = out.step_tokens ? out.step_tokens + k * B * P : g->pred;
    if (seeded) { a.step = i; a.conf_w = nz.conf_weight[i]; }
    else { a.exp_noise = nz.exp_noise + k * B * P * C; a.conf_noise = nz.conf_noise + k * B * P; }
    if (!edit) a.k_mask_len = r.mask_len[i];
    rc = sample_step_checked(kStepEntry[id.kind], a, cur, edit ? g->num_regen : nullptr, edit ? r.mask_ratio[i] : 0.f, s);
    if (rc) return rc;
    last_pred = a.pred;
    int64_t* t = cur; cur = nxt; nxt = t;
  }
  if (s1 < num_steps) {
    if (int rc = launched()) return rc;
    run.next = s1;
    return 0;
  }
  int64_t* codes = out.codes ? out.codes : g->codes;
  mb::combine_groups(s, last_pred, codes, (size_t)B * n, m, g->gbits);
  if (d) {
    int rc = mb_dec_decode(d, codes, out.img_nchw, out.img_nhwc_u8, B, (mb_stream)s);
    if (rc) return rc;
  }
  return launched();
}

int sample_requests_run(mb_gen* g, mb_dec* d, const mb_request_plan& plan, const int64_t* labels, int B, const int64_t* init_tokens, const int64_t* seeds,
                        const RunOut& out, hipStream_t s) {
  const char* who = "mb_sample_requests";
  const int S = plan.num_steps;
  if (!plan.active || !plan.table || !labels || !seeds) return fail(-1, "%s: null argument", who);
  if (S <= 0 || B <= 0) return fail(-1, "%s: bad sizes (num_steps = %d, B = %d)", who, S, B);
  for (int t = 0; t < S; ++t) {
    if (plan.active[t] < 1 || plan.active[t] > B) return fail(-1, "%s: active[%d] = %d outside [1, %d]", who, t, plan.active[t], B);
    if (t && plan.active[t] < plan.active[t - 1])
      return fail(-1, "%s: active[] is not non-decreasing (active[%d] = %d after %d): order the requests by num_steps descending", who, t, plan.active[t], plan.active[t - 1]);
  }
  if (plan.active[S - 1] != B) return fail(-1, "%s: active[%d] = %d, but all %d requests run the last step", who, S - 1, plan.active[S - 1], B);
  if (!d && (out.img_nchw || out.img_nhwc_u8)) return fail(-1, "%s: image requested without a decoder", who);
  if (!g) return fail(-1, "%s: null argument (no generator handle)", who);
  const bool guided = plan.use_guidance != 0;
  const int nbf = guided ? 2 * B : B;
  if (nbf > g->max_seqs) return fail(-1, "%s: B=%d needs %d sequences, engine holds %d", who, B, nbf, g->max_seqs);
  const mb_gen_cfg& c = g->c;
  const int n = c.seq, m = c.splits, C = g->C;
  const size_t P = (size_t)n * m;
  mb_gen::Run& run = g->run;
  run.next = -1;
  if (init_tokens) mb::edit_load_tokens(s, init_tokens, g->tok_a, g->num_regen, B, (int)P, C);
  else {
    mb::fill_i64(s, g->tok_a, (int64_t)C, (size_t)B * P);
    mb::edit_load_tokens(s, g->tok_a, nullptr, g->num_regen, B, (int)P, C);
  }
  HIP_TRY(hipMemcpyAsync(g->tok_b, g->tok_a, (size_t)B * P * sizeof(int64_t), hipMemcpyDeviceToDevice, s));
  int64_t* cur = g->tok_a;
  int64_t* nxt = g->tok_b;
  int64_t* last_pred = g->pred;
  struct CfgReady { mb_gen::Run& run; ~CfgReady() { run.cfg_labels = nullptr; } } cfg_ready{run};
  run.cfg_labels = nullptr;
  mb::StepArgs a{};
  a.logits_c = g->logits; a.P = (int)P; a.C = C;
  a.seeds = seeds;
  for (int t = 0; t < S; ++t) {
    const int Bt = plan.active[t];
    int rc;
    if (guided) {
      rc = gen_forward_cfg(g, cur, labels, g->logits, Bt, s);
      a.logits_u = g->logits + (size_t)Bt * P * C;
      if (Bt <= g->chunk_seqs / 2) { run.cfg_labels = labels; run.cfg_B = Bt; }
      else run.cfg_labels = nullptr;
    } else {
      rc = gen_forward(g, cur, labels, nullptr, g->logits, Bt, s);
      a.logits_u = nullptr;
    }
    if (rc) return rc;
    a.B = Bt;
    a.req = (const mb::RequestStep*)plan.table + (size_t)t * B;
    a.tokens = nxt; a.pred = out.step_tokens ? out.step_tokens + (size_t)t * B * P : g->pred;
    rc = sample_step_checked(who, a, cur, g->num_regen, 0.f, s);
    if (rc) return rc;
    last_pred = a.pred;
    int64_t* tmp = cur; cur = nxt; nxt = tmp;
  }
  int64_t* codes = out.codes ? out.codes : g->codes;
  mb::combine_groups(s, last_pred, codes, (size_t)B * n, m, g->gbits);
  if (d) {
    int rc = mb_dec_decode(d, codes, out.img_nchw, out.img_nhwc_u8, B, (mb_stream)s);
    if (rc) return rc;
  }
  return launched();
}

}

extern "C" {

int mb_sample_requests(mb_gen* g, mb_dec* d, const mb_request_plan* plan, const int64_t* labels, int B, const int64_t* init_tokens, const int64_t* seeds,
                       int64_t* step_tokens, int64_t* tokens_out, float* img_nchw, uint8_t* img_nhwc_u8, mb_stream stream) {
  if (!plan) return fail(-1, "mb_sample_requests: null argument");
  return sample_requests_run(g, d, *plan, labels, B, init_tokens, seeds, RunOut{step_tokens, tokens_out, img_nchw, img_nhwc_u8}, (hipStream_t)stream);
}

int mb_sample(mb_gen* g, mb_dec* d, const mb_sample_plan* plan, const int64_t* labels, int B, const float* exp_noise,
              const float* conf_noise, int64_t* step_tokens, int64_t* tokens_out, float* img_nchw,
              uint8_t* img_nhwc_u8, mb_stream stream) {
  if (!plan || !g || !labels || !exp_noise || !conf_noise) return fail(-1, "mb_sample: null argument");
  RunSpec r = run_spec("mb_sample", *plan);
  r.mask_len = plan->mask_len;
  r.noise.exp_noise = exp_noise; r.noise.conf_noise = conf_noise;
  return sample_run(g, d, r, labels, B, RunOut{step_tokens, tokens_out, img_nchw, img_nhwc_u8}, (hipStream_t)stream);
}

int mb_sample_edit(mb_gen* g, mb_dec* d, const mb_edit_plan* plan, const int64_t* labels, int B, const int64_t* init_tokens, const float* exp_noise,
                   const float* conf_noise, int64_t* step_tokens, int64_t* tokens_out, float* img_nchw, uint8_t* img_nhwc_u8, mb_stream stream) {
  if (!plan || !plan->mask_ratio) return fail(-1, "mb_sample_edit: %s", plan ? "incomplete plan" : "null argument");
  if (!g || !labels || !exp_noise || !conf_noise || !init_tokens) return fail(-1, "mb_sample_edit: null argument");
  RunSpec r = run_spec("mb_sample_edit", *plan);
  r.mask_ratio = plan->mask_ratio;
  r.init_tokens = init_tokens;
  r.noise.exp_noise = exp_noise; r.noise.conf_noise = conf_noise;
  return sample_run(g, d, r, labels, B, RunOut{step_tokens, tokens_out, img_nchw, img_nhwc_u8}, (hipStream_t)stream);
}

int mb_sample_seeded(mb_gen* g, mb_dec* d, const mb_edit_plan* plan, const int64_t* labels, int B, const int64_t* init_tokens, const int64_t* seeds,
                     float randomize_temperature, const float* conf_weight, int64_t* step_tokens, int64_t* tokens_out, float* img_nchw,
                     uint8_t* img_nhwc_u8, mb_stream stream) {
  if (!plan || !plan->mask_ratio) return fail(-1, "mb_sample_seeded: %s", plan ? "incomplete plan" : "null argument");
  if (!seeds || !conf_weight || !g || !labels) return fail(-1, "mb_sample_seeded: null argument");
  RunSpec r = run_spec("mb_sample_seeded", *plan);
  r.mask_ratio = plan->mask_ratio;
  r.init_tokens = init_tokens;
  r.noise.seeds = seeds; r.noise.rand_temp = randomize_temperature; r.noise.conf_weight = conf_weight;
  return sample_run(g, d, r, labels, B, RunOut{step_tokens, tokens_out, img_nchw, img_nhwc_u8}, (hipStream_t)stream);
}

}
```

maskbit_amd/csrc/gemm.hip:

```cpp
#include <cstdio>
#include <cstdlib>

#include "mb_kernels.h"

namespace mb {

constexpr int BM = 128, BN = 128, BK = 64;
constexpr int TILE_BYTES = BM * BK * 2;

template <int EPI>
__global__ __launch_bounds__(256, 2) void gemm_tn_kernel(GemmArgs a) {
  __shared__ __attribute__((aligned(16))) char smem[4 * TILE_BYTES];
  const int tid = threadIdx.x, lane = tid & 63, wave = tid >> 6;
  const int wm = wave >> 1, wn = wave & 1;
  const int tiles_n = (a.N + BN - 1) / BN;
  const int tiles_m = (a.M + BM - 1) / BM;
  const int L = walk_tile(blockIdx.x, tiles_m * tiles_n, a.reverse);
  const int m0 = (L / tiles_n) * BM, n0 = (L % tiles_n) * BN;
  const int K = a.K, KA = a.kw ? a.kw : a.K, nka = KA / BK;
  const int KW = a.kw ? a.kw : a.K, nkw = KW / BK;

  const h16* xsrc[4];
  const h16* wsrc[4];
  const ptrdiff_t a2 = a.A2 ? a.A2 - a.A : 0;
  const ptrdiff_t w2 = a.W2 ? a.W2 - a.W : 0;
#pragma unroll
  for (int j = 0; j < 4; ++j) {
    const int row = wave * 32 + j * 8 + (lane >> 3);
    const int slot = (lane & 7) ^ ((row >> 1) & 7);
    const int mr = min(m0 + row, a.M - 1), nr = min(n0 + row, a.N - 1);
    xsrc[j] = a.A + (size_t)mr * KA + slot * 8;
    wsrc[j] = a.W + (size_t)nr * KW + slot * 8;
  }
  auto stage = [&](int t, int buf) {
    const int ta = t < nka ? t : t - nka;
    char* xb = smem + buf * 2 * TILE_BYTES + wave * 32 * 128;
    char* wb = xb + TILE_BYTES;
    if (a.W2) {
      const int seg = t / nkw, tt = t - seg * nkw;
#pragma unroll
      for (int j = 0; j < 4; ++j) {
        MB_GLDS16(xsrc[j] + (seg == 1 ? a2 : 0) + tt * BK, xb + j * 8 * 128);
        MB_GLDS16(wsrc[j] + (seg == 2 ? w2 : 0) + tt * BK, wb + j * 8 * 128);
      }
      return;
    }
#pragma unroll
    for (int j = 0; j < 4; ++j) {
      MB_GLDS16(xsrc[j] + (t < nka ? 0 : a2) + ta * BK, xb + j * 8 * 128);
      MB_GLDS16(wsrc[j] + (t < nkw ? t : t - nkw) * BK, wb + j * 8 * 128);
    }
  };

  int foff[2];
#pragma unroll
  for (int kk = 0; kk < 2; ++kk)
    foff[kk] = (lane & 15) * 128 + (((kk * 4 + (lane >> 4)) ^ ((lane & 15) >> 1)) * 16);

  f32x4 acc[4][4];
#pragma unroll
  for (int i = 0; i < 4; ++i)
#pragma unroll
    for (int j = 0; j < 4; ++j) acc[i][j] = f32x4{0.f, 0.f, 0.f, 0.f};

  const int nk = K / BK;
  stage(0, 0);
  for (int t = 0; t < nk; ++t) {
    asm volatile("s_waitcnt vmcnt(0)" ::: "memory");
    __syncthreads();
    if (t + 1 < nk) stage(t + 1, (t + 1) & 1);
    const char* xb = smem + (t & 1) * 2 * TILE_BYTES + wm * 64 * 128;
    const char* wb = smem + (t & 1) * 2 * TILE_BYTES + TILE_BYTES + wn * 64 * 128;
#pragma unroll
    for (int kk = 0; kk < 2; ++kk) {
      h16x8 wf[4], xf[4];
#pragma unroll
      for (int i = 0; i < 4; ++i) wf[i] = *(const h16x8*)(wb + i * 16 * 128 + foff[kk]);
#pragma unroll
      for (int j = 0; j < 4; ++j) xf[j] = *(const h16x8*)(xb + j * 16 * 128 + foff[kk]);
#pragma unroll
      for (int i = 0; i < 4; ++i)
#pragma unroll
        for (int j = 0; j < 4; ++j)
          acc[i][j] = MB_MFMA_16x16x32(wf[i], xf[j], acc[i][j]);
    }
  }

  const float sc = a.scale ? *a.scale : 1.0f;
  bool satb = false;
#pragma unroll
  for (int j = 0; j < 4; ++j) {
    const int m = m0 + wm * 64 + j * 16 + (lane & 15);
    if (m >= a.M) continue;
    size_t orow = (size_t)m;
    const float* brow = a.bias;
    if (EPI == EPI_LOGITS_F32) {
      const int sq = m / a.period, pos = m - sq * a.period;
      if (pos == a.period - 1) continue;
      orow = (size_t)sq * (a.period - 1) + pos;
      if (a.bias_per_pos) brow = a.bias + (size_t)pos * a.N;
    }
#pragma unroll
    for (int i = 0; i < 4; ++i) {
      const int n = n0 + wn * 64 + i * 16 + (lane >> 4) * 4;
      if (n >= a.N) continue;
      const float4 b = *(const float4*)(brow + n);
      float v0 = fmaf(acc[i][j][0], sc, b.x), v1 = fmaf(acc[i][j][1], sc, b.y), v2 = fmaf(acc[i][j][2], sc, b.z), v3 = fmaf(acc[i][j][3], sc, b.w);
      if (EPI == EPI_RES_F32) {
        const float4 r = *(const float4*)(a.residual + (size_t)m * a.N + n);
        if (a.ln_stats) {
          const float2 st = *(const float2*)(a.ln_stats + 2 * (size_t)m);
          const float4 g = *(const float4*)(a.ln_g + n), be = *(const float4*)(a.ln_b + n);
          v0 += ln_affine(r.x, st.x, st.y, g.x, be.x); v1 += ln_affine(r.y, st.x, st.y, g.y, be.y);
          v2 += ln_affine(r.z, st.x, st.y, g.z, be.z); v3 += ln_affine(r.w, st.x, st.y, g.w, be.w);
        } else { v0 += r.x; v1 += r.y; v2 += r.z; v3 += r.w; }
      }
      if (EPI == EPI_GELU_H16 || EPI == EPI_GELU_F32) {
        const f32x2 g01 = gelu_erf2((f32x2){v0, v1}), g23 = gelu_erf2((f32x2){v2, v3});
        v0 = g01.x; v1 = g01.y; v2 = g23.x; v3 = g23.y;
      }
      if (EPI == EPI_H16 || EPI == EPI_GELU_H16) {
        satb |= !(fabsf(v0) <= MB_H16_MAX) | !(fabsf(v1) <= MB_H16_MAX) | !(fabsf(v2) <= MB_H16_MAX) | !(fabsf(v3) <= MB_H16_MAX);
        h16x4 o = {to_h(v0), to_h(v1), to_h(v2), to_h(v3)};
        *(h16x4*)(a.out_h16 + orow * a.N + n) = o;
      } else {
        *(float4*)(a.out_f32 + orow * a.N + n) = make_float4(v0, v1, v2, v3);
      }
    }
  }
  if ((EPI == EPI_H16 || EPI == EPI_GELU_H16) && a.sat && satb) atomicAdd(a.sat, 1u);
}

int gemm_tn(hipStream_t s, GemmEpi epi, const GemmArgs& a, int variant) {
  if (a.W2 && (!a.A2 || !a.kw || a.K != 3 * a.kw || !a.scale)) return -1;
  if (variant >= 0 && !a.W2 && gemm_ht_supported(epi, a)) {
    if (variant % 1000 == 257 && a.M % (a.seq_rows ? a.seq_rows : 257)) variant = variant - variant % 1000;
    gemm_ht(s, epi, a, variant);
    return 0;
  }
  if (a.pair_rows || a.nlo) return -1;
  const int tiles = ((a.M + BM - 1) / BM) * ((a.N + BN - 1) / BN);
  dim3 grid(tiles), block(256);
  switch (epi) {
    case EPI_H16: hipLaunchKernelGGL(gemm_tn_kernel<EPI_H16>, grid, block, 0, s, a); break;
    case EPI_GELU_H16: hipLaunchKernelGGL(gemm_tn_kernel<EPI_GELU_H16>, grid, block, 0, s, a); break;
    case EPI_RES_F32: hipLaunchKernelGGL(gemm_tn_kernel<EPI_RES_F32>, grid, block, 0, s, a); break;
    case EPI_GELU_F32: hipLaunchKernelGGL(gemm_tn_kernel<EPI_GELU_F32>, grid, block, 0, s, a); break;
    case EPI_LOGITS_F32: hipLaunchKernelGGL(gemm_tn_kernel<EPI_LOGITS_F32>, grid, block, 0, s, a); break;
  }
  return 0;
}

__global__ void cast_kernel(const float* __restrict__ src, h16* __restrict__ dst, size_t n) {
  size_t i = ((size_t)blockIdx.x * blockDim.x + threadIdx.x) * 4;
  const size_t stride = (size_t)gridDim.x * blockDim.x * 4;
  for (; i + 3 < n; i += stride) {
    const float4 v = *(const float4*)(src + i);
    *(h16x4*)(dst + i) = h16x4{(h16)v.x, (h16)v.y, (h16)v.z, (h16)v.w};
  }
  if (blockIdx.x == 0 && threadIdx.x == 0)
    for (size_t j = n & ~(size_t)3; j < n; ++j) dst[j] = (h16)src[j];
}
void cast_f32_to_h16(hipStream_t s, const float* src, h16* dst, size_t n) {
  const int blocks = (int)min((size_t)2048, (n / 4 + 255) / 256 + 1);
  hipLaunchKernelGGL(cast_kernel, dim3(blocks), dim3(256), 0, s, src, dst, n);
}


__device__ __forceinline__ float half_wave_max(float v) {
#pragma unroll
  for (int o = 16; o > 0; o >>= 1) v = fmaxf(v, __shfl_xor(v, o));
  return v;
}
__device__ __forceinline__ float half_wave_sum(float v) {
#pragma unroll
  for (int o = 16; o > 0; o >>= 1) v += __shfl_xor(v, o);
  return v;
}
__global__ __launch_bounds__(256) void w4_kernel(const float* __restrict__ W, uint8_t* __restrict__ out, int N, int K, uint8_t* __restrict__ scale_out) {
  const int n = blockIdx.x, tid = threadIdx.x;
  const float* w = W + (size_t)n * K;
  const float F4V[8] = {0.f, 0.5f, 1.f, 1.5f, 2.f, 3.f, 4.f, 6.f};
  for (int k = tid * 4; k < K; k += 1024) {
    const float4 v4 = *(const float4*)(w + k);
    const float v[4] = {(float)(h16)v4.x, (float)(h16)v4.y, (float)(h16)v4.z, (float)(h16)v4.w};
    const float rms = sqrtf(half_wave_sum((v[0] * v[0] + v[1] * v[1]) + (v[2] * v[2] + v[3] * v[3])) / 128.0f);
    int r0 = 0;
    if (rms > 0.f && rms < 3.0e38f) r0 = (int)rintf(log2f(2.2f / rms));
    r0 = max(-100, min(100, r0));
    float err[3] = {0.f, 0.f, 0.f};
#pragma unroll
    for (int c = 0; c < 3; ++c) {
      const float m = ldexpf(1.0f, r0 - 1 + c);
#pragma unroll
      for (int e = 0; e < 4; ++e) {
        const float q = F4V[fp4_code(v[e] * m) & 7];
        const float d = fabsf(v[e]) * m - q;
        err[c] += d * d / (m * m);
      }
      err[c] = half_wave_sum(err[c]);
    }
    const int best = (err[1] <= err[0] && err[1] <= err[2]) ? 1 : (err[0] <= err[2] ? 0 : 2);
    const int r = r0 - 1 + best;
    if ((tid & 31) == 0) scale_out[w4_scale_index(n, k >> 7, K)] = (uint8_t)max(0, min(254, 127 - r));
    *(uint16_t*)(out + w4_packed_offset(n, k, K)) = (uint16_t)fp4_pack4(v[0], v[1], v[2], v[3], ldexpf(1.0f, r));
  }
}

__global__ __launch_bounds__(256) void w4lo_kernel(const float* __restrict__ W, uint8_t* __restrict__ out, int N, int K, uint8_t* __restrict__ scale_out) {
  const int n = blockIdx.x, tid = threadIdx.x;
  const float* w = W + (size_t)n * K;
  for (int k = tid * 4; k < K; k += 1024) {
    const float4 v = *(const float4*)(w + k);
    const float e0 = v.x - (float)(h16)v.x, e1 = v.y - (float)(h16)v.y, e2 = v.z - (float)(h16)v.z, e3 = v.w - (float)(h16)v.w;
    const float mx = half_wave_max(fmaxf(fmaxf(fabsf(e0), fabsf(e1)), fmaxf(fabsf(e2), fabsf(e3))));
    if ((tid & 31) == 0) scale_out[w4_scale_index(n, k >> 7, K)] = (uint8_t)fp4_scale_byte_nosat(mx);
    *(uint16_t*)(out + w4_packed_offset(n, k, K)) = (uint16_t)fp4_pack4(e0, e1, e2, e3, fp4_scale_mul_nosat(mx));
  }
}

__global__ void absmax_kernel(const float* __restrict__ src, size_t n, unsigned* __restrict__ out) {
  float m = 0.f;
  for (size_t i = (size_t)blockIdx.x * blockDim.x + threadIdx.x; i < n; i += (size_t)gridDim.x * blockDim.x) m = fmaxf(m, fabsf(src[i]));
  m = wave_max(m);
  if ((threadIdx.x & 63) == 0) atomicMax(out, __float_as_uint(m));
}
__global__ void split_kernel(const float* __restrict__ src, h16* __restrict__ dst, int N, int K, const unsigned* __restrict__ amax,
                             float* __restrict__ scale_out, h16* __restrict__ lo_plane) {
  const float mx = __uint_as_float(*amax);
  int e = 0;
  if (mx > 0.f && mx < 3.0e38f) (void)frexpf(mx, &e);
  const int S = mx > 0.f ? 15 - e : 0;
  if (blockIdx.x == 0 && threadIdx.x == 0) *scale_out = ldexpf(1.0f, -S);
  const size_t n = (size_t)N * K;
  for (size_t i = (size_t)blockIdx.x * blockDim.x + threadIdx.x; i < n; i += (size_t)gridDim.x * blockDim.x) {
    const float w = ldexpf(src[i], S);
    const h16 hi = to_h(w);
    dst[i] = hi; lo_plane[i] = to_h(w - (float)hi);
  }
}
void split_f32_to_h16_planes(hipStream_t s, const float* src, h16* hi, h16* lo, int N, int K, float* scale_out, unsigned* tmp) {
  if (!hi || !lo) abort();
  const size_t n = (size_t)N * K;
  const int blocks = (int)min((size_t)2048, (n + 255) / 256);
  (void)hipMemsetAsync(tmp, 0, sizeof(unsigned), s);
  hipLaunchKernelGGL(absmax_kernel, dim3(blocks), dim3(256), 0, s, src, n, tmp);
  hipLaunchKernelGGL(split_kernel, dim3(blocks), dim3(256), 0, s, src, hi, N, K, tmp, scale_out, lo);
}
void w4_from_f32(hipStream_t s, const float* src, uint8_t* dst4, int N, int K, uint8_t* scale_out) {
  (void)hipMemsetAsync(dst4, 0, (size_t)N * K / 2, s);
  hipLaunchKernelGGL(w4_kernel, dim3(N), dim3(256), 0, s, src, dst4, N, K, scale_out);
}
void w4lo_from_f32(hipStream_t s, const float* src, uint8_t* dst4, int N, int K, uint8_t* scale_out) {
  (void)hipMemsetAsync(dst4, 0, (size_t)N * K / 2, s);
  hipLaunchKernelGGL(w4lo_kernel, dim3(N), dim3(256), 0, s, src, dst4, N, K, scale_out);
}
}
```

maskbit_amd/csrc/mb_kernels.h:

```cpp
#pragma once
#include "mb_common.h"

namespace mb {

enum GemmEpi {
  EPI_H16 = 0,
  EPI_GELU_H16 = 1,
  EPI_RES_F32 = 2,
  EPI_GELU_F32 = 3,
  EPI_LOGITS_F32 = 4,
};
struct GemmArgs {
  const h16* A;
  const h16* W;
  const float* bias;
  const float* residual;
  float* out_f32;
  h16* out_h16;
  int M, N, K;
  int period;
  const float* scale = nullptr;
  const float* ln_stats = nullptr;
  const float* ln_g = nullptr;
  const float* ln_b = nullptr;
  int bias_per_pos = 0;
  const h16* A2 = nullptr;
  int kw = 0;
  const h16* W2 = nullptr;
  int pair_rows = 0;
  int seq_rows = 0;
  uint8_t* out4 = nullptr;
  uint8_t* out4_scale = nullptr;
  uint8_t* out4l = nullptr;
  uint8_t* out4l_scale = nullptr;
  struct LoSet { const uint8_t* A4; const uint8_t* a_scale; const uint8_t* W4; const uint8_t* w_scale; };
  LoSet lo[2] = {};
  int nlo = 0;
  unsigned* sat = nullptr;
  int reverse = 0;
};
__host__ __device__ inline size_t w4_packed_offset(int n, int k, int K) {
  const int r = n & 15, c = (k & 127) >> 5;
  return ((size_t)(n >> 4) * (K >> 7) + (k >> 7)) * 1024 + r * 64 + ((c ^ ((r >> 1) & 3)) << 4) + ((k & 31) >> 1);
}
__host__ __device__ inline size_t w4_scale_index(int n, int j, int K) {
  return (((size_t)(n >> 6) * (K >> 7) + j) * 16 + (n & 15)) * 4 + ((n >> 4) & 3);
}
__host__ __device__ inline size_t fp4_scale_index(int blk, int nseq, int seq, int r, int groups = 4) {
  return (((size_t)blk * nseq + seq) * groups + (r >> 6)) * 64 + (r & 15) * 4 + ((r >> 4) & 3);
}
__host__ __device__ inline int walk_tile(int vb, int ntiles, int reverse) { return xcd_remap(reverse ? ntiles - 1 - vb : vb, ntiles); }
__host__ __device__ inline int xcd_chunk_start(int x, int n) { return xcd_remap(x, n); }
__host__ __device__ inline int walk_seq(int slot, int n, int grp, int reverse) {
  if (reverse) slot = n - 1 - slot;
  const int q = n >> 3, r = n & 7;
  for (int lo = 0, before = 0;; lo += grp) {
    const int a = q + 1 - lo < grp ? (q + 1 - lo > 0 ? q + 1 - lo : 0) : grp;
    const int b = q - lo < grp ? (q - lo > 0 ? q - lo : 0) : grp;
    const int step = r * a + (8 - r) * b;
    if (slot < before + step) {
      int s = slot - before, x;
      if (s < r * a) { x = s / a; s -= x * a; }
      else { s -= r * a; x = s / b; s -= x * b; x += r; }
      return xcd_chunk_start(x, n) + lo + s;
    }
    before += step;
  }
}
inline int walk_group(int seq_rows, bool pair) { const int tps = (seq_rows - 1) / (pair ? 128 : 256); return tps >= 8 ? 1 : tps >= 1 ? 8 / tps : 8; }
struct WalkRows { int seq_rows, grp, reverse; };
__host__ __device__ inline int walk_row(int slot, int rows, const WalkRows& w) {
  if (w.reverse) slot = rows - 1 - slot;
  const int ss = slot / w.seq_rows;
  return walk_seq(ss, rows / w.seq_rows, w.grp, 0) * w.seq_rows + (slot - ss * w.seq_rows);
}
inline WalkRows walk_rows(int rows, int seq_rows, bool pair, int reverse) {
  if (seq_rows <= 0 || rows % seq_rows) return WalkRows{rows, 8, reverse ? 1 : 0};
  return WalkRows{seq_rows, walk_group(seq_rows, pair), reverse ? 1 : 0};
}

int gemm_tn(hipStream_t s, GemmEpi epi, const GemmArgs& a, int variant = 0);
bool gemm_ht_supported(GemmEpi epi, const GemmArgs& a);
void gemm_ht(hipStream_t s, GemmEpi epi, const GemmArgs& a, int mt);
void set_cu_count(int n);

enum GemmF32Epi {
  F32_EPI_PLAIN = 0,
  F32_EPI_GELU = 1,
  F32_EPI_RES = 2,
  F32_EPI_LOGITS = 3,
};
struct GemmF32Args {
  int epi;
  const float* A; const float* W; const float* bias; const float* residual; float* out;
  int M, N, K;
  int period = 0, bias_per_pos = 0;
};
int gemm_f32(hipStream_t s, const GemmF32Args& a);
int attention_f32(hipStream_t s, const float* qkv, float* out, int nb, int N, int d, int heads);

void w4_from_f32(hipStream_t s, const float* src, uint8_t* dst4, int N, int K, uint8_t* scale_out);
void w4lo_from_f32(hipStream_t s, const float* src, uint8_t* dst4, int N, int K, uint8_t* scale_out);

struct Fp4Rows { uint8_t* x4 = nullptr; uint8_t* x4s = nullptr; uint8_t* xl4 = nullptr; uint8_t* xl4s = nullptr; int nseq = 0; int seq_rows = 257; };

void layernorm_rows(hipStream_t s, const float* y, const float* gamma, const float* beta, float eps,
                    float* x_f32, h16* x_h16, float* stats, int M, int d, h16* x_lo = nullptr,
                    const Fp4Rows& f4 = Fp4Rows{}, int reverse = 0, int seq_rows = 0);

int layernorm_pair(hipStream_t s, const float* y, const float* gamma, const float* beta, float eps, h16* x_h16, float* stats, int P, int d,
                   const Fp4Rows& f4 = Fp4Rows{}, int reverse = 0, int seq_rows = 0);
int pairify_rows(hipStream_t s, const float* x32, h16* x_h16, int P, int d, const Fp4Rows& f4 = Fp4Rows{}, int reverse = 0, int seq_rows = 0);

struct EmbedArgs {
  const int64_t* tokens;
  const int64_t* labels;
  const uint8_t* drop;
  const float* w_in;
  const float* b_in;
  const float* class_emb;
  const float* pos;
  const float* gamma; const float* beta;
  float* x_f32; h16* x_h16;
  int nb, seq, m, gbits, d, nclass;
  const float* tables = nullptr;
  h16* x_lo = nullptr;
  Fp4Rows f4;
};
void embed_ln(hipStream_t s, const EmbedArgs& a);
int embed_pair(hipStream_t s, const EmbedArgs& a);
void transpose_f32(hipStream_t s, const float* src , float* dst , int rows, int cols);

void attention(hipStream_t s, const h16* qkv, h16* out, int nb, int N, int d, int heads,
               uint8_t* out4 = nullptr, uint8_t* out4s = nullptr, int reverse = 0);
int attention_pair(hipStream_t s, const h16* qkv, h16* out, int P, int N, int d, int heads, uint8_t* out4 = nullptr, uint8_t* out4s = nullptr,
                   uint8_t* out4l = nullptr, uint8_t* out4ls = nullptr, int reverse = 0);
int attention_probs(hipStream_t s, const h16* qkv, float* out, int nb, int N, int d, int heads);

struct RequestStep { float scale, temperature, mask_ratio, rand_temp, conf_w; int32_t step; };
struct StepArgs {
  const float* logits_c; const float* logits_u;
  float scale, temperature;
  const float* exp_noise;
  const float* conf_noise;
  int k_mask_len;
  int64_t* tokens;
  int64_t* pred;
  int B, P , C;
  const int64_t* seeds = nullptr;
  int step = 0;
  float rand_temp = 0.f, conf_w = 0.f;
  const RequestStep* req = nullptr;
};
int sample_step(hipStream_t s, const StepArgs& a, const int64_t* tokens_in, const int* num_regen = nullptr, float mask_ratio = 0.f);
int seeded_noise_dump(hipStream_t s, const int64_t* seeds, int step, float rand_temp, float conf_w, float* exp_u, float* exp_noise, float* conf_u,
                      float* conf_noise, int B, int P, int C);

void fill_i64(hipStream_t s, int64_t* dst, int64_t value, size_t n);

void edit_load_tokens(hipStream_t s, const int64_t* src, int64_t* dst, int* num_regen, int B, int P, int C);
void edit_init(hipStream_t s, const int64_t* codes, const uint8_t* regen, int64_t* tokens, int* num_regen, int B, int n, int m, int gbits);
void edit_token_mask(hipStream_t s, const uint8_t* pixel_mask, uint8_t* token_mask, int B, int H, int W, int st);
int edit_composite(hipStream_t s, const float* gen, const float* orig, const uint8_t* pixel_mask, float* out_nchw, uint8_t* out_u8, int B, int C, int H, int W);
void combine_groups(hipStream_t s, const int64_t* tokens , int64_t* codes , size_t rows, int m, int gbits);

void cast_f32_to_h16(hipStream_t s, const float* src, h16* dst, size_t n);
void split_f32_to_h16_planes(hipStream_t s, const float* src, h16* hi, h16* lo, int N, int K, float* scale_out, unsigned* tmp);

}
```

maskbit_amd/csrc/norm_embed.hip:

```cpp
#include "mb_kernels.h"

namespace mb {

constexpr int MAXS = 32;

template <int NV>
__device__ __forceinline__ void fp4_row_store(const float4* v, int lane, uint8_t* x4row, uint8_t* scales, int nseq, int seq, int tok, int groups) {
#pragma unroll
  for (int q = 0; q < NV; ++q) {
    float am = fmaxf(fmaxf(fabsf(v[q].x), fabsf(v[q].y)), fmaxf(fabsf(v[q].z), fabsf(v[q].w)));
    am = row16_max(am);
    if ((lane & 15) == 0) scales[fp4_scale_index(q * 4 + (lane >> 4), nseq, seq, tok, groups)] = (uint8_t)fp4_scale_byte_nosat(am);
    *(uint16_t*)(x4row + q * 128 + lane * 2) = (uint16_t)fp4_pack4(v[q].x, v[q].y, v[q].z, v[q].w, fp4_scale_mul_nosat(am));
  }
}
template <int NV>
__device__ __forceinline__ void fp4_rows_out(const Fp4Rows& f4, float4* v, int lane, int row, int d) {
  const int seq = row / f4.seq_rows, tok = row - seq * f4.seq_rows, groups = (f4.seq_rows - 1) >> 6;
  if (tok == f4.seq_rows - 1) return;
  if (f4.x4) fp4_row_store<NV>(v, lane, f4.x4 + (size_t)row * 2 * d, f4.x4s, f4.nseq, seq, tok, groups);
  if (f4.xl4) {
#pragma unroll
    for (int q = 0; q < NV; ++q)
      v[q] = make_float4(v[q].x - (float)to_h(v[q].x), v[q].y - (float)to_h(v[q].y), v[q].z - (float)to_h(v[q].z), v[q].w - (float)to_h(v[q].w));
    fp4_row_store<NV>(v, lane, f4.xl4 + (size_t)row * 2 * d, f4.xl4s, f4.nseq, seq, tok, groups);
  }
}

template <int NV>
__device__ __forceinline__ void ln_finish(float4* v, const float* sc, int ns, int d, int lane,
                                          const float* __restrict__ gamma, const float* __restrict__ beta,
                                          float eps, float* xo, h16* xb, float* st = nullptr, h16* xl = nullptr,
                                          const Fp4Rows* f4 = nullptr, int row = 0) {
  constexpr bool VEC = NV > 0;
  constexpr int nv = NV;
  float s = 0.f;
  if (VEC) {
#pragma unroll
    for (int q = 0; q < nv; ++q) s += (v[q].x + v[q].y) + (v[q].z + v[q].w);
  }
  else     { for (int q = 0; q < ns; ++q) s += sc[q]; }
  const float mean = wave_sum(s) / (float)d;
  float ss = 0.f;
  if (VEC) {
#pragma unroll
    for (int q = 0; q < nv; ++q) {
      const float a = v[q].x - mean, b = v[q].y - mean, c = v[q].z - mean, e = v[q].w - mean;
      ss += (a * a + b * b) + (c * c + e * e);
    }
  } else {
    for (int q = 0; q < ns; ++q) { const int c = lane + q * 64; if (c < d) { const float a = sc[q] - mean; ss += a * a; } }
  }
  const float rstd = rsqrtf(wave_sum(ss) / (float)d + eps);
  if (st && lane == 0) *(float2*)st = make_float2(mean, rstd);
  if (VEC) {
#pragma unroll
    for (int q = 0; q < nv; ++q) {
      const int c = q * 256 + lane * 4;
      const float4 g = *(const float4*)(gamma + c), b = *(const float4*)(beta + c);
      float4 o;
      o.x = ln_affine(v[q].x, mean, rstd, g.x, b.x); o.y = ln_affine(v[q].y, mean, rstd, g.y, b.y);
      o.z = ln_affine(v[q].z, mean, rstd, g.z, b.z); o.w = ln_affine(v[q].w, mean, rstd, g.w, b.w);
      if (xo) *(float4*)(xo + c) = o;
      const h16x4 hi = {to_h(o.x), to_h(o.y), to_h(o.z), to_h(o.w)};
      if (xb) *(h16x4*)(xb + c) = hi;
      if (xl) *(h16x4*)(xl + c) = h16x4{to_h(o.x - (float)hi[0]), to_h(o.y - (float)hi[1]), to_h(o.z - (float)hi[2]), to_h(o.w - (float)hi[3])};
      if (f4) v[q] = o;
    }
    if constexpr (VEC) { if (f4) fp4_rows_out<NV>(*f4, v, lane, row, d); }
  } else {
    for (int q = 0; q < ns; ++q) {
      const int c = lane + q * 64;
      if (c < d) {
        const float o = ln_affine(sc[q], mean, rstd, gamma[c], beta[c]);
        if (xo) xo[c] = o;
        if (xb) xb[c] = to_h(o);
        if (xl) xl[c] = to_h(o - (float)to_h(o));
      }
    }
  }
}

template <int NV>
__global__ __launch_bounds__(256) void ln_rows_kernel(const float* __restrict__ y, const float* __restrict__ gamma,
                                                      const float* __restrict__ beta, float eps, float* x_f32,
                                                      h16* x_h16, float* stats, int M, int d, h16* x_lo, Fp4Rows f4, WalkRows wk) {
  const int lane = threadIdx.x & 63;
  const int slot = blockIdx.x * 4 + __builtin_amdgcn_readfirstlane(threadIdx.x >> 6);
  if (slot >= M) return;
  const int row = walk_row(slot, M, wk);
  const float* yr = y + (size_t)row * d;
  constexpr bool VEC = NV > 0;
  float4 v[VEC ? NV : 1]; float sc[VEC ? 1 : MAXS];
  const int ns = (d + 63) / 64;
  if (VEC) {
#pragma unroll
    for (int q = 0; q < NV; ++q) v[q] = *(const float4*)(yr + q * 256 + lane * 4);
  }
  else     { for (int q = 0; q < ns; ++q) { const int c = lane + q * 64; sc[q] = c < d ? yr[c] : 0.f; } }
  ln_finish<NV>(v, sc, ns, d, lane, gamma, beta, eps, x_f32 ? x_f32 + (size_t)row * d : nullptr,
                 x_h16 ? x_h16 + (size_t)row * d : nullptr, stats ? stats + (size_t)row * 2 : nullptr,
                 x_lo ? x_lo + (size_t)row * d : nullptr,
                 (f4.x4 || f4.xl4) ? &f4 : nullptr, row);
}

template <int NV>
__device__ __forceinline__ float2 ln_normalize(float4* v, int d, const float* __restrict__ gamma, const float* __restrict__ beta, float eps, int lane) {
  float s = 0.f;
#pragma unroll
  for (int q = 0; q < NV; ++q) s += (v[q].x + v[q].y) + (v[q].z + v[q].w);
  const float mean = wave_sum(s) / (float)d;
  float ss = 0.f;
#pragma unroll
  for (int q = 0; q < NV; ++q) {
    const float a = v[q].x - mean, b = v[q].y - mean, c = v[q].z - mean, e = v[q].w - mean;
    ss += (a * a + b * b) + (c * c + e * e);
  }
  const float rstd = rsqrtf(wave_sum(ss) / (float)d + eps);
#pragma unroll
  for (int q = 0; q < NV; ++q) {
    const int c = q * 256 + lane * 4;
    const float4 g = *(const float4*)(gamma + c), b = *(const float4*)(beta + c);
    v[q] = make_float4(ln_affine(v[q].x, mean, rstd, g.x, b.x), ln_affine(v[q].y, mean, rstd, g.y, b.y),
                       ln_affine(v[q].z, mean, rstd, g.z, b.z), ln_affine(v[q].w, mean, rstd, g.w, b.w));
  }
  return make_float2(mean, rstd);
}

template <int NV>
__device__ __forceinline__ void pair_store(float4* xc, const float4* xu, int lane, h16* oc, h16* ou, const Fp4Rows& f4, int row, int d) {
#pragma unroll
  for (int q = 0; q < NV; ++q) {
    const int c = q * 256 + lane * 4;
    *(h16x4*)(oc + c) = h16x4{to_h(xc[q].x), to_h(xc[q].y), to_h(xc[q].z), to_h(xc[q].w)};
    *(h16x4*)(ou + c) = h16x4{to_h(xu[q].x - xc[q].x), to_h(xu[q].y - xc[q].y), to_h(xu[q].z - xc[q].z), to_h(xu[q].w - xc[q].w)};
  }
  if (f4.x4 || f4.xl4) fp4_rows_out<NV>(f4, xc, lane, row, d);
}

template <int NV>
__global__ __launch_bounds__(256) void ln_pair_kernel(const float* __restrict__ y, const float* __restrict__ gamma, const float* __restrict__ beta, float eps,
                                                      h16* __restrict__ x_h16, float* __restrict__ stats, int P, int d, Fp4Rows f4, WalkRows wk) {
  const int lane = threadIdx.x & 63;
  const int slot = blockIdx.x * 4 + __builtin_amdgcn_readfirstlane(threadIdx.x >> 6);
  if (slot >= P) return;
  const int row = walk_row(slot, P, wk);
  float4 vc[NV], vu[NV];
#pragma unroll
  for (int q = 0; q < NV; ++q) { vc[q] = *(const float4*)(y + (size_t)row * d + q * 256 + lane * 4); vu[q] = *(const float4*)(y + (size_t)(row + P) * d + q * 256 + lane * 4); }
  const float2 sc = ln_normalize<NV>(vc, d, gamma, beta, eps, lane), su = ln_normalize<NV>(vu, d, gamma, beta, eps, lane);
  if (stats && lane == 0) { *(float2*)(stats + 2 * (size_t)row) = sc; *(float2*)(stats + 2 * (size_t)(row + P)) = su; }
  pair_store<NV>(vc, vu, lane, x_h16 + (size_t)row * d, x_h16 + (size_t)(row + P) * d, f4, row, d);
}

template <int NV>
__global__ __launch_bounds__(256) void pairify_kernel(const float* __restrict__ x32, h16* __restrict__ x_h16, int P, int d, Fp4Rows f4, WalkRows wk) {
  const int lane = threadIdx.x & 63;
  const int slot = blockIdx.x * 4 + __builtin_amdgcn_readfirstlane(threadIdx.x >> 6);
  if (slot >= P) return;
  const int row = walk_row(slot, P, wk);
  float4 vc[NV], vu[NV];
#pragma unroll
  for (int q = 0; q < NV; ++q) { vc[q] = *(const float4*)(x32 + (size_t)row * d + q * 256 + lane * 4); vu[q] = *(const float4*)(x32 + (size_t)(row + P) * d + q * 256 + lane * 4); }
  pair_store<NV>(vc, vu, lane, x_h16 + (size_t)row * d, x_h16 + (size_t)(row + P) * d, f4, row, d);
}

int layernorm_pair(hipStream_t s, const float* y, const float* gamma, const float* beta, float eps, h16* x_h16, float* stats, int P, int d,
                   const Fp4Rows& f4, int reverse, int seq_rows) {
  dim3 grid((P + 3) / 4), block(256);
  const WalkRows wk = walk_rows(P, seq_rows, true, reverse);
  if (d == 1024) hipLaunchKernelGGL(ln_pair_kernel<4>, grid, block, 0, s, y, gamma, beta, eps, x_h16, stats, P, d, f4, wk);
  else if (d == 768) hipLaunchKernelGGL(ln_pair_kernel<3>, grid, block, 0, s, y, gamma, beta, eps, x_h16, stats, P, d, f4, wk);
  else return -1;
  return 0;
}
int pairify_rows(hipStream_t s, const float* x32, h16* x_h16, int P, int d, const Fp4Rows& f4, int reverse, int seq_rows) {
  dim3 grid((P + 3) / 4), block(256);
  const WalkRows wk = walk_rows(P, seq_rows, true, reverse);
  if (d == 1024) hipLaunchKernelGGL(pairify_kernel<4>, grid, block, 0, s, x32, x_h16, P, d, f4, wk);
  else if (d == 768) hipLaunchKernelGGL(pairify_kernel<3>, grid, block, 0, s, x32, x_h16, P, d, f4, wk);
  else return -1;
  return 0;
}

void layernorm_rows(hipStream_t s, const float* y, const float* gamma, const float* beta, float eps,
                    float* x_f32, h16* x_h16, float* stats, int M, int d, h16* x_lo, const Fp4Rows& f4, int reverse, int seq_rows) {
  dim3 grid((M + 3) / 4), block(256);
  const WalkRows wk = walk_rows(M, seq_rows, false, reverse);
  if (d == 1024) hipLaunchKernelGGL(ln_rows_kernel<4>, grid, block, 0, s, y, gamma, beta, eps, x_f32, x_h16, stats, M, d, x_lo, f4, wk);
  else if (d == 768) hipLaunchKernelGGL(ln_rows_kernel<3>, grid, block, 0, s, y, gamma, beta, eps, x_f32, x_h16, stats, M, d, x_lo, f4, wk);
  else hipLaunchKernelGGL(ln_rows_kernel<0>, grid, block, 0, s, y, gamma, beta, eps, x_f32, x_h16, stats, M, d, x_lo, Fp4Rows{}, wk);
}

constexpr int MAXBITS = 24;

template <int NV>
__global__ __launch_bounds__(256) void embed_ln_kernel(EmbedArgs a) {
  const int lane = threadIdx.x & 63;
  const int row = blockIdx.x * 4 + (threadIdx.x >> 6);
  const int N = a.seq + 1;
  if (row >= a.nb * N) return;
  const int sq = row / N, t = row - sq * N;
  const int d = a.d, K = a.m * a.gbits;
  uint32_t plus = 0, live = 0;
  const float* cls = nullptr;
  const float* trow[8] = {};
  if (t < a.seq) {
    for (int g = 0; g < a.m; ++g) {
      const int64_t idx = a.tokens[((size_t)sq * a.seq + t) * a.m + g];
      if (a.tables && g < 8) {
        const int64_t nrow = ((int64_t)1 << a.gbits) + 1;
        const int64_t ix = idx < 0 ? 0 : (idx >= nrow ? nrow - 1 : idx);
        trow[g] = a.tables + ((size_t)g * nrow + (size_t)ix) * d;
      }
      const uint32_t gm = (1u << a.gbits) - 1u;
      if (idx != ((int64_t)1 << a.gbits)) { live |= gm << (g * a.gbits); plus |= ((uint32_t)idx & gm) << (g * a.gbits); }
    }
  } else {
    int64_t lab = a.labels[sq];
    if (a.drop && a.drop[sq]) lab = a.nclass;
    lab = lab < 0 ? 0 : (lab > a.nclass ? a.nclass : lab);
    cls = a.class_emb + (size_t)lab * d;
  }
  const float* pos = a.pos + (size_t)t * d;
  constexpr bool VEC = NV > 0;
  float4 v[VEC ? NV : 1]; float sc[VEC ? 1 : MAXS];
  const int ns = (d + 63) / 64;
  if (VEC) {
#pragma unroll
    for (int q = 0; q < NV; ++q) {
      const int c = q * 256 + lane * 4;
      float4 e = cls ? *(const float4*)(cls + c) : (a.tables ? make_float4(0.f, 0.f, 0.f, 0.f) : *(const float4*)(a.b_in + c));
      if (!cls && a.tables) {
#pragma unroll
        for (int g = 0; g < 8; ++g)
          if (g < a.m) { const float4 w = *(const float4*)(trow[g] + c); e.x += w.x; e.y += w.y; e.z += w.z; e.w += w.w; }
      } else if (!cls) {
#pragma unroll
        for (int j = 0; j < MAXBITS; ++j) {
          if (j < K) {
            const float4 w = *(const float4*)(a.w_in + (size_t)j * d + c);
            const float sj = ((live >> j) & 1u) ? (((plus >> j) & 1u) ? 1.f : -1.f) : 0.f;
            e.x = fmaf(sj, w.x, e.x); e.y = fmaf(sj, w.y, e.y); e.z = fmaf(sj, w.z, e.z); e.w = fmaf(sj, w.w, e.w);
          }
        }
      }
      const float4 p = *(const float4*)(pos + c);
      v[q] = make_float4(e.x + p.x, e.y + p.y, e.z + p.z, e.w + p.w);
    }
  } else {
    for (int q = 0; q < ns; ++q) {
      const int c = lane + q * 64;
      float e = 0.f;
      if (c < d) {
        if (cls) e = cls[c];
        else if (a.tables) {
          for (int g = 0; g < a.m && g < 8; ++g) e += trow[g][c];
        } else {
          e = a.b_in[c];
          for (int j = 0; j < K; ++j) {
            const float sj = ((live >> j) & 1u) ? (((plus >> j) & 1u) ? 1.f : -1.f) : 0.f;
            e = fmaf(sj, a.w_in[(size_t)j * d + c], e);
          }
        }
        e += pos[c];
      }
      sc[q] = e;
    }
  }
  ln_finish<NV>(v, sc, ns, d, lane, a.gamma, a.beta, 1e-12f, a.x_f32 + (size_t)row * d, a.x_h16 ? a.x_h16 + (size_t)row * d : nullptr, nullptr,
                 a.x_lo ? a.x_lo + (size_t)row * d : nullptr,
                 (a.f4.x4 || a.f4.xl4) ? &a.f4 : nullptr, row);
}

template <int NV>
__global__ __launch_bounds__(256) void embed_pair_kernel(EmbedArgs a) {
  const int lane = threadIdx.x & 63;
  const int row = blockIdx.x * 4 + (threadIdx.x >> 6);
  const int N = a.seq + 1, P = a.nb * N;
  if (row >= P) return;
  const int sq = row / N, t = row - sq * N;
  const int d = a.d, K = a.m * a.gbits;
  uint32_t plus = 0, live = 0;
  const float* cls = nullptr;
  if (t < a.seq) {
    for (int g = 0; g < a.m; ++g) {
      const int64_t idx = a.tokens[((size_t)sq * a.seq + t) * a.m + g];
      const uint32_t gm = (1u << a.gbits) - 1u;
      if (idx != ((int64_t)1 << a.gbits)) { live |= gm << (g * a.gbits); plus |= ((uint32_t)idx & gm) << (g * a.gbits); }
    }
  } else {
    int64_t lab = a.labels[sq];
    lab = lab < 0 ? 0 : (lab > a.nclass ? a.nclass : lab);
    cls = a.class_emb + (size_t)lab * d;
  }
  const float* pos = a.pos + (size_t)t * d;
  float4 vc[NV], vu[NV];
#pragma unroll
  for (int q = 0; q < NV; ++q) {
    const int c = q * 256 + lane * 4;
    float4 e = cls ? *(const float4*)(cls + c) : *(const float4*)(a.b_in + c);
    if (!cls) {
#pragma unroll
      for (int j = 0; j < MAXBITS; ++j) {
        if (j < K) {
          const float4 w = *(const float4*)(a.w_in + (size_t)j * d + c);
          const float sj = ((live >> j) & 1u) ? (((plus >> j) & 1u) ? 1.f : -1.f) : 0.f;
          e.x = fmaf(sj, w.x, e.x); e.y = fmaf(sj, w.y, e.y); e.z = fmaf(sj, w.z, e.z); e.w = fmaf(sj, w.w, e.w);
        }
      }
    }
    const float4 p = *(const float4*)(pos + c);
    vc[q] = make_float4(e.x + p.x, e.y + p.y, e.z + p.z, e.w + p.w);
    if (cls) {
      const float4 eu = *(const float4*)(a.class_emb + (size_t)a.nclass * d + c);
      vu[q] = make_float4(eu.x + p.x, eu.y + p.y, eu.z + p.z, eu.w + p.w);
    }
  }
  ln_normalize<NV>(vc, d, a.gamma, a.beta, 1e-12f, lane);
  if (cls) ln_normalize<NV>(vu, d, a.gamma, a.beta, 1e-12f, lane);
  else {
#pragma unroll
    for (int q = 0; q < NV; ++q) vu[q] = vc[q];
  }
#pragma unroll
  for (int q = 0; q < NV; ++q) {
    const int c = q * 256 + lane * 4;
    *(float4*)(a.x_f32 + (size_t)row * d + c) = vc[q];
    *(float4*)(a.x_f32 + (size_t)(row + P) * d + c) = vu[q];
  }
  pair_store<NV>(vc, vu, lane, a.x_h16 + (size_t)row * d, a.x_h16 + (size_t)(row + P) * d, a.f4, row, d);
}

int embed_pair(hipStream_t s, const EmbedArgs& a) {
  if (a.tables || a.m * a.gbits > MAXBITS) return -1;
  const int rows = a.nb * (a.seq + 1);
  dim3 grid((rows + 3) / 4), block(256);
  if (a.d == 1024) hipLaunchKernelGGL(embed_pair_kernel<4>, grid, block, 0, s, a);
  else if (a.d == 768) hipLaunchKernelGGL(embed_pair_kernel<3>, grid, block, 0, s, a);
  else return -1;
  return 0;
}

void embed_ln(hipStream_t s, const EmbedArgs& a) {
  const int rows = a.nb * (a.seq + 1);
  dim3 grid((rows + 3) / 4), block(256);
  if (a.d == 1024) hipLaunchKernelGGL(embed_ln_kernel<4>, grid, block, 0, s, a);
  else if (a.d == 768) hipLaunchKernelGGL(embed_ln_kernel<3>, grid, block, 0, s, a);
  else hipLaunchKernelGGL(embed_ln_kernel<0>, grid, block, 0, s, a);
}

__global__ void transpose_f32_kernel(const float* __restrict__ src, float* __restrict__ dst, int rows, int cols) {
  const int i = blockIdx.x * blockDim.x + threadIdx.x;
  if (i < rows * cols) { const int r = i / cols, c = i - r * cols; dst[(size_t)c * rows + r] = src[i]; }
}
void transpose_f32(hipStream_t s, const float* src, float* dst, int rows, int cols) {
  hipLaunchKernelGGL(transpose_f32_kernel, dim3((rows * cols + 255) / 256), dim3(256), 0, s, src, dst, rows, cols);
}

}
```

Before: 34.99.

## Compact final layernorm and head GEMMs to rows still masked

Adds a device-side row map of positions that still hold a mask token, and runs the last layernorm and both head GEMMs only over those compacted rows. The logits GEMM scatters its output back to the original positions. This skips head work for already-decoded tokens that the sampling step never reads. It adds two small kernels per forward, a device-read extent inside the GEMM, and a heuristic that disables pruning when most positions are still masked. Unmasked rows' logits are left stale, which is only correct if sampling truly ignores them.

```diff
diff --git a/include/maskbit_hip_diag.h b/include/maskbit_hip_diag.h
--- a/include/maskbit_hip_diag.h
+++ b/include/maskbit_hip_diag.h
@@ -55,6 +55,9 @@
 int mb_walk_seq(int slot, int n, int grp, int reverse);
 int mb_walk_row(int slot, int rows, int seq_rows, int pair, int reverse);
 int mb_walk_group(int seq_rows, int pair);
+int mb_gen_set_prune(mb_gen* g, int mode);
+int mb_gen_forward_cfg_pruned(mb_gen* g, const int64_t* tokens, const int64_t* labels, float* logits, int B, mb_stream stream);
+int mb_gen_pruned_rows(mb_gen* g, int* rows, mb_stream stream);
 int mb_gemm_ht_supported(int epi, int M, int N, int K);
 
 int mb_seeded_noise(const int64_t* seeds, int step, float randomize_temperature, float conf_weight, float* exp_u, float* exp_noise, float* conf_u,
diff --git a/maskbit_amd/_lib.py b/maskbit_amd/_lib.py
--- a/maskbit_amd/_lib.py
+++ b/maskbit_amd/_lib.py
@@ -171,6 +171,9 @@
     "mb_set_cu_count":(C.c_int, [C.c_int]),
     "mb_gen_set_walk": (C.c_int, [C.c_void_p, C.c_int]),
     "mb_diag_set_walk": (C.c_int, [C.c_int]),
+    "mb_gen_set_prune": (C.c_int, [C.c_void_p, C.c_int]),
+    "mb_gen_forward_cfg_pruned": (C.c_int, [C.c_void_p, C.c_void_p, C.c_void_p, C.c_void_p, C.c_int, C.c_void_p]),
+    "mb_gen_pruned_rows": (C.c_int, [C.c_void_p, C.POINTER(C.c_int), C.c_void_p]),
     "mb_walk_tile": (C.c_int, [C.c_int] * 3),
     "mb_walk_seq": (C.c_int, [C.c_int] * 4),
     "mb_walk_row": (C.c_int, [C.c_int] * 5),
diff --git a/maskbit_amd/build.py b/maskbit_amd/build.py
--- a/maskbit_amd/build.py
+++ b/maskbit_amd/build.py
@@ -8,7 +8,7 @@
 HERE = os.path.dirname(os.path.abspath(__file__))
 CSRC = os.path.join(HERE, "csrc")
 LIB = os.path.join(HERE, "libmaskbit_hip.so")
-SOURCES = ["engine.hip", "diag.hip", "gemm.hip", "gemm_ht.hip", "gemm_f32.hip", "norm_embed.hip", "attention.hip", "sampling.hip", "edit.hip", "conv.hip", "decoder.hip", "vq.hip", "evaluator.hip", "mlm.hip", "lpips.hip", "fid.hip", "manifold.hip", "inception.hip", "spatial_attention.hip", "taming.hip"]
+SOURCES = ["engine.hip", "diag.hip", "gemm.hip", "gemm_ht.hip", "gemm_f32.hip", "norm_embed.hip", "compact.hip", "attention.hip", "sampling.hip", "edit.hip", "conv.hip", "decoder.hip", "vq.hip", "evaluator.hip", "mlm.hip", "lpips.hip", "fid.hip", "manifold.hip", "inception.hip", "spatial_attention.hip", "taming.hip"]
 
 
 def hipcc() -> str:
diff --git a/maskbit_amd/csrc/compact.hip b/maskbit_amd/csrc/compact.hip
--- /dev/null
+++ b/maskbit_amd/csrc/compact.hip
@@ -0,0 +1,54 @@
+#include "mb_kernels.h"
+
+namespace mb {
+
+__device__ __forceinline__ bool position_masked(const int64_t* __restrict__ tok, int m, int64_t mask_tok) {
+  bool any = false;
+  for (int g = 0; g < m; ++g) any |= tok[g] == mask_tok;
+  return any;
+}
+
+__global__ __launch_bounds__(256) void prune_count_kernel(const int64_t* __restrict__ tokens, int seq, int m, int64_t mask_tok, int* __restrict__ counts) {
+  __shared__ int wsum[4];
+  const int b = blockIdx.x, tid = threadIdx.x;
+  int cnt = 0;
+  for (int p = tid; p < seq; p += 256) cnt += position_masked(tokens + ((size_t)b * seq + p) * m, m, mask_tok);
+  cnt = (int)wave_sum((float)cnt);
+  if ((tid & 63) == 0) wsum[tid >> 6] = cnt;
+  __syncthreads();
+  if (tid == 0) counts[b] = wsum[0] + wsum[1] + wsum[2] + wsum[3];
+}
+
+__global__ __launch_bounds__(256) void prune_map_kernel(const int64_t* __restrict__ tokens, int B, int seq, int m, int64_t mask_tok,
+                                                        const int* __restrict__ counts, int* __restrict__ rows, int* __restrict__ extent) {
+  __shared__ int wsum[4];
+  const int b = blockIdx.x, tid = threadIdx.x, lane = tid & 63, wave = tid >> 6;
+  int base = 0, R = 0;
+  for (int i = 0; i < B; ++i) { const int c = counts[i]; base += i < b ? c : 0; R += c; }
+  if (b == 0 && tid == 0) *extent = 2 * R;
+  const int N = seq + 1, P = B * N;
+  int run = base;
+  for (int p0 = 0; p0 < seq; p0 += 256) {
+    const int p = p0 + tid;
+    const bool masked = p < seq && position_masked(tokens + ((size_t)b * seq + p) * m, m, mask_tok);
+    const unsigned long long bal = __ballot(masked);
+    if (lane == 0) wsum[wave] = __popcll(bal);
+    __syncthreads();
+    int off = run, tot = 0;
+    for (int w = 0; w < 4; ++w) { off += w < wave ? wsum[w] : 0; tot += wsum[w]; }
+    if (masked) {
+      const int j = off + __popcll(bal & ((1ull << lane) - 1ull));
+      rows[j] = b * N + p;
+      rows[R + j] = P + b * N + p;
+    }
+    run += tot;
+    __syncthreads();
+  }
+}
+
+void prune_row_map(hipStream_t s, const int64_t* tokens, int B, int seq, int m, int64_t mask_tok, int* counts, int* rows, int* extent) {
+  hipLaunchKernelGGL(prune_count_kernel, dim3(B), dim3(256), 0, s, tokens, seq, m, mask_tok, counts);
+  hipLaunchKernelGGL(prune_map_kernel, dim3(B), dim3(256), 0, s, tokens, B, seq, m, mask_tok, counts, rows, extent);
+}
+
+}
diff --git a/maskbit_amd/csrc/engine.hip b/maskbit_amd/csrc/engine.hip
--- a/maskbit_amd/csrc/engine.hip
+++ b/maskbit_amd/csrc/engine.hip
@@ -56,6 +56,9 @@
   int* num_regen = nullptr;
   int alo_mask = 0, alo_mask_built = 0;
   int walk = 1;
+  int prune = 1;
+  bool prune_ok = false;
+  int *prune_counts = nullptr, *prune_rows = nullptr, *prune_ext = nullptr;
   bool f32 = false;
   struct Layer32 { float *wqkv = nullptr, *wo = nullptr, *w1 = nullptr, *w2 = nullptr; };
   std::vector<Layer32> layers32;
@@ -75,7 +78,7 @@
   m.zeroed(&b->s, (width / 64) * ntok + 256);
 }
 
-int head_gemms(mb_gen* g, float* logits, int M, hipStream_t s) {
+int head_gemms(mb_gen* g, float* logits, int M, hipStream_t s, bool compact = false) {
   using namespace mb;
   const mb_gen_cfg& c = g->c;
   const int d = c.hidden;
@@ -83,13 +86,16 @@
   { ProfScope p("gemm_head", s, true);
     GemmArgs ga{g->x_h16, g->wl, g->bl, nullptr, g->y_f32, nullptr, M, d, 3 * d, 0, g->head_scale};
     ga.A2 = g->x_lo; ga.kw = d; ga.W2 = g->wl_lo;
+    if (compact) ga.m_extent = g->prune_ext;
     rc |= gemm_tn(s, EPI_GELU_F32, ga); }
   { ProfScope p("layernorm", s, true);
-    layernorm_rows(s, g->y_f32, g->lnhg, g->lnhb, 1e-12f, nullptr, g->x_h16, nullptr, M, d, g->x_lo); }
+    if (compact) rc |= layernorm_rows_compact(s, g->y_f32, g->lnhg, g->lnhb, 1e-12f, g->x_h16, g->x_lo, M, d, g->prune_ext, nullptr);
+    else layernorm_rows(s, g->y_f32, g->lnhg, g->lnhb, 1e-12f, nullptr, g->x_h16, nullptr, M, d, g->x_lo); }
   { ProfScope p("gemm_head", s, true);
     GemmArgs ga{g->x_h16, g->wp, c.embed_tables ? g->bias_pos : g->bp, nullptr, logits, nullptr, M, c.splits * g->C, (g->wp_lo ? 3 : 2) * d, g->N,
                 g->wp_lo ? g->head_scale + 1 : nullptr};
     ga.A2 = g->x_lo; ga.kw = d; ga.W2 = g->wp_lo;
+    if (compact) { ga.m_extent = g->prune_ext; ga.out_rows = g->prune_rows; }
     ga.bias_per_pos = c.embed_tables;
     rc |= gemm_tn(s, EPI_LOGITS_F32, ga); }
   return rc;
@@ -171,7 +177,8 @@
   return 0;
 }
 
-int gen_forward_pair_impl(mb_gen* g, const int64_t* tokens, const int64_t* labels, const uint8_t* drop, float* logits, int B, bool wmode, hipStream_t s) {
+int gen_forward_pair_impl(mb_gen* g, const int64_t* tokens, const int64_t* labels, const uint8_t* drop, float* logits, int B, bool wmode, hipStream_t s,
+                          bool prune = false) {
   using namespace mb;
   const mb_gen_cfg& c = g->c;
   const int d = c.hidden, f = c.mlp, N = g->N, nb = 2 * B, M = nb * N, P = B * N;
@@ -210,6 +217,10 @@
       embed_ln(s, e);
       rc |= pairify_rows(s, g->y_f32, g->x_h16, P, d, f4_for(), walk_next(), N);
     }
+  }
+  if (prune) {
+    ProfScope p("prune_map", s, true);
+    prune_row_map(s, tokens, B, c.seq, c.splits, (int64_t)g->C, g->prune_counts, g->prune_rows, g->prune_ext);
   }
   if (c.prenorm && c.depth > 0) {
     ProfScope p("layernorm", s, true);
@@ -244,10 +255,12 @@
         if (l + 1 == c.depth) layernorm_rows(s, g->y_f32, g->lnag, g->lnab, 1e-12f, nullptr, g->x_h16, nullptr, M, d, g->x_lo, Fp4Rows{}, walk_next(), N);
         else rc |= layernorm_pair(s, g->y_f32, g->layers[l + 1].ln1g, g->layers[l + 1].ln1b, 1e-12f, g->x_h16, nullptr, P, d, f4_for(), walk_next(), N);
       }
+      else if (l + 1 == c.depth && prune)
+        rc |= layernorm_rows_compact(s, g->y_f32, L.ln2g, L.ln2b, 1e-12f, g->x_h16, g->x_lo, M, d, g->prune_ext, g->prune_rows);
       else if (l + 1 == c.depth) layernorm_rows(s, g->y_f32, L.ln2g, L.ln2b, 1e-12f, nullptr, g->x_h16, g->ln_stats, M, d, g->x_lo, Fp4Rows{}, walk_next(), N);
       else rc |= layernorm_pair(s, g->y_f32, L.ln2g, L.ln2b, 1e-12f, g->x_h16, g->ln_stats, P, d, f4_for(), walk_next(), N); }
   }
-  rc |= head_gemms(g, logits, M, s);
+  rc |= head_gemms(g, logits, M, s, prune);
   if (int lrc = launched()) return lrc;
   if (rc) return fail(-3, "differential CFG forward: a kernel refused the shape (%d pairs x %d tokens, hidden %d, mlp %d)", B, N, d, f);
   return 0;
@@ -316,9 +329,10 @@
   return 0;
 }
 
-int gen_forward_cfg(mb_gen* g, const int64_t* tokens, const int64_t* labels, float* logits, int B, hipStream_t s) {
+int gen_forward_cfg(mb_gen* g, const int64_t* tokens, const int64_t* labels, float* logits, int B, hipStream_t s, bool prune = false) {
   const size_t P = (size_t)g->c.seq * g->c.splits;
   const bool pair = !g->f32 && g->pair_ok && g->c.precision >= 1;
+  prune = prune && pair && g->prune_ok && g->c.depth > 0;
   const bool wmode = pair && g->c.precision >= 2;
   const int chunk = g->chunk_seqs / 2;
   if (chunk < 1) return fail(-1, "engine holds %d sequences: too few for a guided forward", g->chunk_seqs);
@@ -335,7 +349,7 @@
     }
     float* out = (nc == B) ? logits : g->logits_tmp;
     if (b0 == 0) g_prof.begin_forward(false);
-    int rc = pair ? gen_forward_pair_impl(g, g->tok_cfg, g->lab_cfg, g->drop_cfg, out, nc, wmode, s)
+    int rc = pair ? gen_forward_pair_impl(g, g->tok_cfg, g->lab_cfg, g->drop_cfg, out, nc, wmode, s, prune)
                   : gen_forward_pass(g, g->tok_cfg, g->lab_cfg, g->drop_cfg, out, 2 * nc, s);
     if (rc) return rc;
     if (nc != B) {
@@ -455,6 +469,8 @@
   m.get(&g->lab_cfg, B); m.get(&g->drop_cfg, B); m.get(&g->logits, B * P * C);
   m.get(&g->num_regen, B);
   if (g->chunk_seqs < max_seqs) m.get(&g->logits_tmp, (size_t)g->chunk_seqs * P * C);
+  g->prune_ok = g->pair_ok && !c.prenorm && !c.embed_tables;
+  if (g->prune_ok) { m.get(&g->prune_counts, (size_t)g->chunk_seqs); m.get(&g->prune_rows, M); m.zeroed(&g->prune_ext, 1); }
   if (int rc = m.failed("mb_gen_create")) { delete g; return rc; }
   *out = g;
   return 0;
@@ -566,6 +582,27 @@
   return 0;
 }
 
+int mb_gen_set_prune(mb_gen* g, int mode) {
+  if (!g || (mode != 0 && mode != 1)) return fail(-1, "mb_gen_set_prune: mode 0 (every row) or 1 (the rows the sampling step reads)");
+  g->prune = mode;
+  return 0;
+}
+
+int mb_gen_forward_cfg_pruned(mb_gen* g, const int64_t* tokens, const int64_t* labels, float* logits, int B, mb_stream stream) {
+  if (!g || !tokens || !labels || !logits) return fail(-1, "mb_gen_forward_cfg_pruned: null argument");
+  if (B <= 0 || 2 * B > g->max_seqs) return fail(-1, "mb_gen_forward_cfg_pruned: B=%d needs %d sequences, engine holds %d", B, 2 * B, g->max_seqs);
+  return gen_forward_cfg(g, tokens, labels, logits, B, (hipStream_t)stream, true);
+}
+
+int mb_gen_pruned_rows(mb_gen* g, int* rows, mb_stream stream) {
+  if (!g || !rows) return fail(-1, "mb_gen_pruned_rows: null argument");
+  *rows = -1;
+  if (!g->prune_ok) return 0;
+  HIP_TRY(hipMemcpyAsync(rows, g->prune_ext, sizeof(int), hipMemcpyDeviceToHost, (hipStream_t)stream));
+  HIP_TRY(hipStreamSynchronize((hipStream_t)stream));
+  return 0;
+}
+
 int mb_gen_saturation_count(mb_gen* g, unsigned* count, int reset, mb_stream stream) {
   if (!g || !count) return fail(-1, "mb_gen_saturation_count: null argument");
   HIP_TRY(hipMemcpyAsync(count, g->sat, sizeof(unsigned), hipMemcpyDeviceToHost, (hipStream_t)stream));
@@ -718,10 +755,19 @@
   mb::StepArgs a{};
   a.logits_c = g->logits; a.B = B; a.P = (int)P; a.C = C;
   a.seeds = nz.seeds; a.rand_temp = nz.rand_temp;
+  auto prune_step = [&](int i) {
+    if (!g->prune) return false;
+    if (r.init_tokens) return true;
+    if (i == 0) return false;
+    const double f = edit ? (double)r.mask_ratio[i - 1] : (double)r.mask_len[i - 1] / (double)P;
+    double keep = 1.0;
+    for (int q = 0; q < m; ++q) keep *= 1.0 - std::min(std::max(f, 0.0), 1.0);
+    return keep > 0.03;
+  };
   for (int i = s0; i < s1; ++i) {
     int rc;
     if (id.guided && (r.scale[i] != 0.0f || (!g->f32 && g->pair_ok && c.precision >= 4))) {
-      rc = gen_forward_cfg(g, cur, labels, g->logits, B, s);
+      rc = gen_forward_cfg(g, cur, labels, g->logits, B, s, prune_step(i));
       a.logits_u = g->logits + (size_t)B * P * C;
       if (B <= g->chunk_seqs / 2) { run.cfg_labels = labels; run.cfg_B = B; }
     } else {
@@ -794,7 +840,7 @@
     const int Bt = plan.active[t];
     int rc;
     if (guided) {
-      rc = gen_forward_cfg(g, cur, labels, g->logits, Bt, s);
+      rc = gen_forward_cfg(g, cur, labels, g->logits, Bt, s, g->prune && (t > 0 || init_tokens));
       a.logits_u = g->logits + (size_t)Bt * P * C;
       if (Bt <= g->chunk_seqs / 2) { run.cfg_labels = labels; run.cfg_B = Bt; }
       else run.cfg_labels = nullptr;
diff --git a/maskbit_amd/csrc/gemm.hip b/maskbit_amd/csrc/gemm.hip
--- a/maskbit_amd/csrc/gemm.hip
+++ b/maskbit_amd/csrc/gemm.hip
@@ -8,13 +8,15 @@
 constexpr int BM = 128, BN = 128, BK = 64;
 constexpr int TILE_BYTES = BM * BK * 2;
 
-template <int EPI>
-__global__ __launch_bounds__(256, 2) void gemm_tn_kernel(GemmArgs a) {
+template <int EPI, bool EXT>
+__device__ __forceinline__ void gemm_tn_body(const GemmArgs& a) {
   __shared__ __attribute__((aligned(16))) char smem[4 * TILE_BYTES];
   const int tid = threadIdx.x, lane = tid & 63, wave = tid >> 6;
   const int wm = wave >> 1, wn = wave & 1;
   const int tiles_n = (a.N + BN - 1) / BN;
-  const int tiles_m = (a.M + BM - 1) / BM;
+  const int m_act = EXT ? min(max(*a.m_extent, 0), a.M) : a.M;
+  const int tiles_m = (m_act + BM - 1) / BM;
+  if (EXT && (int)blockIdx.x >= tiles_m * tiles_n) return;
   const int L = walk_tile(blockIdx.x, tiles_m * tiles_n, a.reverse);
   const int m0 = (L / tiles_n) * BM, n0 = (L % tiles_n) * BN;
   const int K = a.K, KA = a.kw ? a.kw : a.K, nka = KA / BK;
@@ -91,11 +93,12 @@
 #pragma unroll
   for (int j = 0; j < 4; ++j) {
     const int m = m0 + wm * 64 + j * 16 + (lane & 15);
-    if (m >= a.M) continue;
+    if (m >= m_act) continue;
     size_t orow = (size_t)m;
     const float* brow = a.bias;
     if (EPI == EPI_LOGITS_F32) {
-      const int sq = m / a.period, pos = m - sq * a.period;
+      const int mf = (EXT && a.out_rows) ? a.out_rows[m] : m;
+      const int sq = mf / a.period, pos = mf - sq * a.period;
       if (pos == a.period - 1) continue;
       orow = (size_t)sq * (a.period - 1) + pos;
       if (a.bias_per_pos) brow = a.bias + (size_t)pos * a.N;
@@ -130,10 +133,15 @@
   }
   if ((EPI == EPI_H16 || EPI == EPI_GELU_H16) && a.sat && satb) atomicAdd(a.sat, 1u);
 }
+template <int EPI>
+__global__ __launch_bounds__(256, 2) void gemm_tn_kernel(GemmArgs a) { gemm_tn_body<EPI, false>(a); }
+template <int EPI>
+__global__ __launch_bounds__(256, 2) void gemm_tn_ext_kernel(GemmArgs a) { gemm_tn_body<EPI, true>(a); }
 
 int gemm_tn(hipStream_t s, GemmEpi epi, const GemmArgs& a, int variant) {
   if (a.W2 && (!a.A2 || !a.kw || a.K != 3 * a.kw || !a.scale)) return -1;
-  if (variant >= 0 && !a.W2 && gemm_ht_supported(epi, a)) {
+  if (a.out_rows && !a.m_extent) return -1;
+  if (variant >= 0 && !a.W2 && !a.m_extent && gemm_ht_supported(epi, a)) {
     if (variant % 1000 == 257 && a.M % (a.seq_rows ? a.seq_rows : 257)) variant = variant - variant % 1000;
     gemm_ht(s, epi, a, variant);
     return 0;
@@ -141,6 +149,12 @@
   if (a.pair_rows || a.nlo) return -1;
   const int tiles = ((a.M + BM - 1) / BM) * ((a.N + BN - 1) / BN);
   dim3 grid(tiles), block(256);
+  if (a.m_extent) {
+    if (epi == EPI_GELU_F32) hipLaunchKernelGGL(gemm_tn_ext_kernel<EPI_GELU_F32>, grid, block, 0, s, a);
+    else if (epi == EPI_LOGITS_F32) hipLaunchKernelGGL(gemm_tn_ext_kernel<EPI_LOGITS_F32>, grid, block, 0, s, a);
+    else return -1;
+    return 0;
+  }
   switch (epi) {
     case EPI_H16: hipLaunchKernelGGL(gemm_tn_kernel<EPI_H16>, grid, block, 0, s, a); break;
     case EPI_GELU_H16: hipLaunchKernelGGL(gemm_tn_kernel<EPI_GELU_H16>, grid, block, 0, s, a); break;
diff --git a/maskbit_amd/csrc/mb_kernels.h b/maskbit_amd/csrc/mb_kernels.h
--- a/maskbit_amd/csrc/mb_kernels.h
+++ b/maskbit_amd/csrc/mb_kernels.h
@@ -38,6 +38,8 @@
   int nlo = 0;
   unsigned* sat = nullptr;
   int reverse = 0;
+  const int* m_extent = nullptr;
+  const int* out_rows = nullptr;
 };
 __host__ __device__ inline size_t w4_packed_offset(int n, int k, int K) {
   const int r = n & 15, c = (k & 127) >> 5;
@@ -108,6 +110,10 @@
                     float* x_f32, h16* x_h16, float* stats, int M, int d, h16* x_lo = nullptr,
                     const Fp4Rows& f4 = Fp4Rows{}, int reverse = 0, int seq_rows = 0);
 
+void prune_row_map(hipStream_t s, const int64_t* tokens, int B, int seq, int m, int64_t mask_tok, int* counts, int* rows, int* extent);
+int layernorm_rows_compact(hipStream_t s, const float* y, const float* gamma, const float* beta, float eps, h16* x_h16, h16* x_lo, int M, int d,
+                           const int* extent, const int* src_rows);
+
 int layernorm_pair(hipStream_t s, const float* y, const float* gamma, const float* beta, float eps, h16* x_h16, float* stats, int P, int d,
                    const Fp4Rows& f4 = Fp4Rows{}, int reverse = 0, int seq_rows = 0);
 int pairify_rows(hipStream_t s, const float* x32, h16* x_h16, int P, int d, const Fp4Rows& f4 = Fp4Rows{}, int reverse = 0, int seq_rows = 0);
diff --git a/maskbit_amd/csrc/norm_embed.hip b/maskbit_amd/csrc/norm_embed.hip
--- a/maskbit_amd/csrc/norm_embed.hip
+++ b/maskbit_amd/csrc/norm_embed.hip
@@ -84,12 +84,14 @@
 template <int NV>
 __global__ __launch_bounds__(256) void ln_rows_kernel(const float* __restrict__ y, const float* __restrict__ gamma,
                                                       const float* __restrict__ beta, float eps, float* x_f32,
-                                                      h16* x_h16, float* stats, int M, int d, h16* x_lo, Fp4Rows f4, WalkRows wk) {
+                                                      h16* x_h16, float* stats, int M, int d, h16* x_lo, Fp4Rows f4, WalkRows wk,
+                                                      const int* __restrict__ extent = nullptr, const int* __restrict__ src_rows = nullptr) {
   const int lane = threadIdx.x & 63;
   const int slot = blockIdx.x * 4 + __builtin_amdgcn_readfirstlane(threadIdx.x >> 6);
   if (slot >= M) return;
-  const int row = walk_row(slot, M, wk);
-  const float* yr = y + (size_t)row * d;
+  if (extent && slot >= *extent) return;
+  const int row = extent ? slot : walk_row(slot, M, wk);
+  const float* yr = y + (size_t)((extent && src_rows) ? src_rows[slot] : row) * d;
   constexpr bool VEC = NV > 0;
   float4 v[VEC ? NV : 1]; float sc[VEC ? 1 : MAXS];
   const int ns = (d + 63) / 64;
@@ -187,9 +189,19 @@
                     float* x_f32, h16* x_h16, float* stats, int M, int d, h16* x_lo, const Fp4Rows& f4, int reverse, int seq_rows) {
   dim3 grid((M + 3) / 4), block(256);
   const WalkRows wk = walk_rows(M, seq_rows, false, reverse);
-  if (d == 1024) hipLaunchKernelGGL(ln_rows_kernel<4>, grid, block, 0, s, y, gamma, beta, eps, x_f32, x_h16, stats, M, d, x_lo, f4, wk);
-  else if (d == 768) hipLaunchKernelGGL(ln_rows_kernel<3>, grid, block, 0, s, y, gamma, beta, eps, x_f32, x_h16, stats, M, d, x_lo, f4, wk);
-  else hipLaunchKernelGGL(ln_rows_kernel<0>, grid, block, 0, s, y, gamma, beta, eps, x_f32, x_h16, stats, M, d, x_lo, Fp4Rows{}, wk);
+  if (d == 1024) hipLaunchKernelGGL(ln_rows_kernel<4>, grid, block, 0, s, y, gamma, beta, eps, x_f32, x_h16, stats, M, d, x_lo, f4, wk, (const int*)nullptr, (const int*)nullptr);
+  else if (d == 768) hipLaunchKernelGGL(ln_rows_kernel<3>, grid, block, 0, s, y, gamma, beta, eps, x_f32, x_h16, stats, M, d, x_lo, f4, wk, (const int*)nullptr, (const int*)nullptr);
+  else hipLaunchKernelGGL(ln_rows_kernel<0>, grid, block, 0, s, y, gamma, beta, eps, x_f32, x_h16, stats, M, d, x_lo, Fp4Rows{}, wk, (const int*)nullptr, (const int*)nullptr);
+}
+
+int layernorm_rows_compact(hipStream_t s, const float* y, const float* gamma, const float* beta, float eps, h16* x_h16, h16* x_lo, int M, int d,
+                           const int* extent, const int* src_rows) {
+  dim3 grid((M + 3) / 4), block(256);
+  const WalkRows wk = walk_rows(M, 0, false, 0);
+  if (d == 1024) hipLaunchKernelGGL(ln_rows_kernel<4>, grid, block, 0, s, y, gamma, beta, eps, (float*)nullptr, x_h16, (float*)nullptr, M, d, x_lo, Fp4Rows{}, wk, extent, src_rows);
+  else if (d == 768) hipLaunchKernelGGL(ln_rows_kernel<3>, grid, block, 0, s, y, gamma, beta, eps, (float*)nullptr, x_h16, (float*)nullptr, M, d, x_lo, Fp4Rows{}, wk, extent, src_rows);
+  else return -1;
+  return 0;
 }
 
 constexpr int MAXBITS = 24;
```

Result: no change. 35.06, median of 6 (+0.2%).
